# Wendison/FCL-taco2

Measured on AMD Instinct MI355X. Metric: mel-frames/sec (FCL-taco2-S forward, batch=32, 80-mel), higher is better.
Workload: dtype f32 via bf16x3-split MFMA operands, fp32 accumulate (max-abs 8e-6 on mel vs the reference; FCL_PRECISION=0 = exact fp32 MFMA)

## Files before the change

fcl-taco2_amd/_lib.py:

```python
import ctypes as C
import os

_HERE = os.path.dirname(os.path.abspath(__file__))
LIB_PATH = os.environ.get("FCL_LIB") or os.path.join(_HERE, "libfcl_hip.so")

_P = C.c_void_p
_I = C.c_int
_F = C.c_float
_Z = C.c_size_t


class DecoderWeights(C.Structure):
    _fields_ = [("c", _I), ("p", _I), ("u", _I), ("odim", _I)] + [
        (n, _P) for n in ("prenet_w0", "prenet_b0", "prenet_w1", "prenet_b1", "w0_att", "w0_pre", "w0_pos", "w0_hh", "b0",
                          "w1_ih", "w1_hh", "b1", "wf_h", "wf_att")
    ] + [("zoneout_rate", _F), ("prenet_dropout", _F)] + [
        (n + sfx, _P) for n in ("prenet_w0", "prenet_w1", "w0_pre", "w0_hh", "w1_ih", "w1_hh", "wf_h") for sfx in ("_hi", "_lo")] + [
        (n + "_p", _P) for n in ("w0_att", "wf_att", "w0_pre", "w0_hh", "w1_ih", "w1_hh")] + [("out_act", _I), ("wf_h_ff", _P), ("prenet_w0_ff", _P), ("prenet_w1_ff", _P),
                                                                                           ("w0_pre_ff", _P), ("w0_hh_ff", _P), ("w1_ih_ff", _P), ("w1_hh_ff", _P), ("stream", _P),
                                                                                           ("prenet_layers", _I), ("dlayers", _I), ("prenet_w2", _P), ("prenet_b2", _P), ("w2_ih", _P),
                                                                                           ("w2_hh", _P), ("b2", _P), ("reduction_factor", _I)]


class DecoderIO(C.Structure):
# ... 84 lines not shown
        (n, _P) for n in ("window", "twiddle", "frame_utt", "utt_off", "utt_seed", "s", "p", "fr", "y", "c_prev", "c_out", "u_out")]


class Features(C.Structure):
    _fields_ = [("frames", C.c_int64), ("samples", C.c_int64)] + [(n, C.c_int32) for n in ("n_fft", "hop", "n_utt", "n_mels", "nnz", "reserved")] + [
        (n, _P) for n in ("x", "smp_off", "frame_utt", "utt_off", "window", "twiddle", "fb_lo", "fb_off", "fb_w", "mel_stats", "mel", "energy", "mag_out")]


class Pitch(C.Structure):
    _fields_ = [("frames", C.c_int64), ("samples", C.c_int64)] + [(n, C.c_int32) for n in ("n", "hop", "n_utt", "tau_min", "tau_max", "reserved")] + [
        ("fs", _F), ("threshold", _F)] + [(n, _P) for n in ("x", "smp_off", "frame_utt", "utt_off", "f0", "cmnd_out", "tau_out")]


class Resample(C.Structure):
    _fields_ = [("samples_in", C.c_int64), ("samples_out", C.c_int64)] + [(n, C.c_int32) for n in ("l", "m", "k", "n_utt", "max_out", "reserved")] + [
        (n, _P) for n in ("x", "smp_off_in", "smp_off_out", "table", "y")]


class Evaluate(C.Structure):
    _fields_ = [(n, C.c_int64) for n in ("frames_a", "frames_b", "cells", "path_rows")] + [(n, C.c_int32) for n in ("n_pairs", "d", "max_ta", "max_tb")] + [
        (n, _P) for n in ("a", "b", "a_off", "b_off", "cell_off", "path_off", "workspace")] + [("workspace_bytes", _Z)] + [
        (n, _P) for n in ("path", "path_len", "cost", "pitch_a", "pitch_b", "counts", "sums")]


class Align(C.Structure):
    _fields_ = [(n, C.c_int64) for n in ("frames", "rows", "cells")] + [(n, C.c_int32) for n in ("n_utt", "n_states", "max_t", "max_s", "max_skip", "reserved")] + [
        (n, _P) for n in ("ll", "frame_off", "row_off", "cell_off", "row_state", "row_skip", "workspace")] + [("workspace_bytes", _Z)] + [
        (n, _P) for n in ("frame_row", "row_begin", "row_frames", "score", "ok")]


class StftLoss(C.Structure):
    _fields_ = [("frames", C.c_int64), ("samples", C.c_int64)] + [(n, C.c_int32) for n in ("n_fft", "hop", "n_utt", "accumulate")] + [
        (n, _P) for n in ("x", "y", "smp_off", "frame_utt", "utt_off", "window", "twiddle", "frame_sums", "utt_sums", "coef", "fr", "gx")]


class MelLoss(C.Structure):
    _fields_ = [("frames", C.c_int64), ("samples", C.c_int64)] + [(n, C.c_int32) for n in ("n_fft", "hop", "n_utt", "accumulate", "n_mels", "nnz")] + [
        (n, _P) for n in ("x", "y", "smp_off", "frame_utt", "utt_off", "window", "twiddle", "fb_lo", "fb_off", "fb_w", "bt_off", "bt_ch", "bt_w",
                          "frame_sums", "utt_sums", "coef", "fr", "gx")]


class PwdLayer(C.Structure):
    _fields_ = [("samples", C.c_int64)] + [(n, C.c_int32) for n in ("cin", "cout", "ksize", "dilation")] + [("slope", _F), ("reserved", C.c_int32)] + [
        (n, _P) for n in ("x", "w", "bias", "h", "g", "seg_lo", "seg_hi", "y", "dw", "db", "workspace")] + [("workspace_bytes", _Z)]


class BernoulliSite(C.Structure):
    _fields_ = [("out", _P), ("n", C.c_int64), ("p_one", _F), ("seed", C.c_uint32)]


BERNOULLI_MAX_SITES = 16


class LossTerm(C.Structure):
    _fields_ = [(n, _P) for n in ("a", "b", "b2", "valid", "valid2", "da", "da_planes", "sums", "sums2")] + [
        ("m", C.c_int32), ("c", C.c_int32), ("b_log", C.c_int32), ("b_log_offset", _F), ("w_l1", _F), ("w_mse", _F), ("count", C.c_double),
        ("w_l1_2", _F), ("w_mse_2", _F), ("count2", C.c_double)]


LOSS_MAX_TERMS, SUM_ROWS_MAX = 12, 6


class ProfEntry(C.Structure):
    _fields_ = [("name", C.c_char * 56), ("launches", _I), ("ms", C.c_double), ("flops", C.c_double), ("rows", C.c_double), ("fill_bytes", C.c_double)]


TE_MAX_SITES, TE_MAX_LOSSES = 48, 48
TE_TEACHER, TE_KD_TEACHER, TE_STUDENT = 0, 1, 2


class TeConfig(C.Structure):
    _fields_ = ([(n, C.c_int32) for n in ("role", "idim", "odim", "embed_dim", "econv_layers", "econv_chans", "econv_filts", "eunits", "dunits", "prenet_units",
                                          "postnet_layers", "postnet_chans", "postnet_filts", "dp_layers", "dp_chans", "dp_kernel", "vp_layers", "vp_chans",
                                          "vp_kernel", "ve_kernel")]
                + [(n, _F) for n in ("dropout_rate", "zoneout_rate", "dp_dropout", "vp_dropout", "ve_dropout")]
                + [(n, C.c_int32) for n in ("use_masking", "t_embed_dim", "t_econv_chans", "t_eunits", "t_prenet_units", "t_dunits", "t_postnet_chans", "share_proj",
                                            "distill_output", "distill_encoder", "distill_decoder", "distill_prosody", "accum_grad")]
                + [("seed", C.c_uint32), ("site_tag", C.c_uint32 * TE_MAX_SITES), ("dw_planes_min", C.c_int32), ("pred_stream", C.c_int32),
                   ("late_losses", C.c_int32)])


class TeBatch(C.Structure):
    _fields_ = ([(n, C.c_int32) for n in ("B", "T", "L", "N", "F", "lmax")]
                + [(n, _P) for n in ("xs", "ys", "f0", "energy", "ds", "lens", "e_lo", "e_hi", "f_lo", "f_hi", "src_sorted", "row_of_enc", "cell_frame", "frame_cell",
                                     "prev_frame", "cell_row", "dur", "perm_tb", "cell_row_i64", "enc_pad", "enc_valid", "frame_valid", "cell_valid", "pos4",
                                     "live_rows_host")]
                + [("n_enc", C.c_double), ("n_frames", C.c_double)])


class TeKnowledge(C.Structure):
    _fields_ = [("after", _P), ("before", _P), ("enc", _P * 5), ("dec", _P * 8), ("pro", _P * 5), ("dec_cell_major", C.c_int32)]


SIGNATURES = {
    "fcl_te_create": (_I, [C.POINTER(TeConfig), C.POINTER(_P)]),
    "fcl_te_destroy": (None, [_P]),
    "fcl_te_site_name": (C.c_char_p, [_I]),
    "fcl_te_loss_name": (C.c_char_p, [_I]),
    "fcl_te_bind_param": (_I, [_P, C.c_char_p, _P, _P, C.c_int64]),
    "fcl_te_bind_buffer": (_I, [_P, C.c_char_p, _P]),
    "fcl_te_finalize": (_I, [_P, _P]),
    "fcl_te_params_changed": (_I, [_P]),
    "fcl_te_side_stream": (_P, [_P]),
    "fcl_te_place_streams": (_I, [_P, _P, C.POINTER(C.c_int)]),
    "fcl_te_knowledge": (_I, [_P, C.POINTER(TeBatch), C.c_uint32, C.POINTER(TeKnowledge), _P]),
    "fcl_te_forward_backward": (_I, [_P, C.POINTER(TeBatch), C.POINTER(TeKnowledge), C.c_uint32, _P, _P, _P]),
    "fcl_te_backward_stage": (_I, [_P, _I, _P]),
    "fcl_te_join": (_I, [_P, _P]),
    "fcl_te_last_launches": (C.c_int64, [_P]),
    "fcl_te_phase_ms": (_I, [_P, _P]),
    "fcl_te_arena_bytes": (C.c_int64, [_P]),
    "fcl_last_error": (C.c_char_p, []),
    "fcl_version": (_I, []),
    "fcl_debug_ptr": (_P, []),
    "fcl_set_gemm_mode": (_I, [_I]),
    "fcl_get_gemm_mode": (_I, []),
    "fcl_pack_conv1d_weight": (_I, [_P, _P, _P, _I, _I, _I, _P]),
    "fcl_fold_batchnorm": (_I, [_P, _P, _P, _P, _F, _P, _P, _I, _P]),
    "fcl_copy2d": (_I, [_P, _I, _P, _I, _I, _I, _P]),
    "fcl_add2d": (_I, [_P, _I, _P, _I, _I, _I, _F, _P, _P]),
    "fcl_frag_bf16_elems": (_Z, [_I, _I]),
    "fcl_pack_frag_bf16": (_I, [_P, _I, _I, _P, _P, _P]),
    "fcl_pack_frag_f32": (_I, [_P, _I, _I, _P, _P]),
    "fcl_add_vec": (_I, [_P, _P, _P, _I, _P]),
    "fcl_u32_add": (_I, [_P, C.c_uint32, _P]),
    "fcl_planes_elems": (_Z, [_I, _I]),
    "fcl_pack_planes": (_I, [_P, _I, _I, _I, _P, _P]),
    "fcl_linear_planes_fwd": (_I, [_P, _I, _P, _P, _P, _I, _P, _I, _I, _I, _I, _P]),
    "fcl_linear_planes_mse_fwd": (_I, [_P, _I, _P, _P, _I, _P, C.c_double, _P, _I, _P, _P, _I, _I, _I, _P]),
    "fcl_conv1d_planes_fwd": (_I, [_P, _I, _P, _P, _P, _P, _P, _P, _P, _I, _I, _I, _I, _I, _P]),
    "fcl_conv1d_planes_rows_fwd": (_I, [_P, _I, _P, _P, _P, _P, _P, _P, _P, _I, _I, _I, _I, _I, _P, _P]),
    "fcl_embedding_fwd": (_I, [_P, _P, _P, _P, _I, _I, _I, _P]),
    "fcl_embed_conv_table_fwd": (_I, [_P] * 8 + [_I, _I, _I, _I, _I, _P, _P]),
    "fcl_linear_fwd": (_I, [_P, _I, _P, _I, _P, _P, _I, _I, _I, _I, _I, _P]),
    "fcl_conv1d_fwd": (_I, [_P, _P, _P, _P, _P, _P, _P, _I, _I, _I, _I, _I, _P]),
    "fcl_layernorm_fwd": (_I, [_P, _P, _P, _F, _P, _P, _P, _P, _P, _P, _F, _P, _I, _I, _P]),
    "fcl_layernorm_group_fwd": (_I, [_P, _I, C.c_int64, _P, _P, _F, _P, _P, _P, _P, _P, _P, _I, _I, _I, _P]),
    "fcl_conv1d_planes_bn_fwd": (_I, [_P, _I, _P, _P, _P, _P, _I, _I, _I, _I, C.c_float, C.c_float, _P, _P, _P, _P, _P, _P]),
    "fcl_conv1d_planes_group_fwd": (_I, [_P, _I, C.c_int64, _P, _P, _P, _P, _P, _P, _I, _I, _I, _I, _I, _I, _P]),
    "fcl_duration_round_fwd": (_I, [_P, _P, _I, _I, _F, _P, _P]),
    "fcl_variance_embed_add_fwd": (_I, [_P] * 12 + [_I, _I, _I, _P]),
    "fcl_duration_round_ctl_fwd": (_I, [_P, _P, _I, _I, _F, _P, _P, _I, _I, _P]),
    "fcl_variance_embed_add_ctl_fwd": (_I, [_P] * 10 + [_I, _I] + [_P] * 5 + [_I, _I, _I, _P]),
    "fcl_variance_embed_rows_fwd": (_I, [_P] * 11 + [_I, _I] + [_P] * 3 + [_I, _I, _I, _I, _P]),
    "fcl_position_table_fwd": (_I, [_P, _P, _I, _I, _P]),
    "fcl_concat_spk_fwd": (_I, [_P, _I, _P, _P, _P, _I, _I, _I, _I, _P]),
    "fcl_kaldi_ark_append": (C.c_longlong, [_I, C.c_longlong, _I, _P, _P, _P, _I, _P]),
    "fcl_host_device_ptr": (_P, [_P]),
    "fcl_feed_copy": (_I, [_P, _P, _Z, _P, _P, _P, _P]),
    "fcl_row_maps_build": (_I, [C.POINTER(RowMaps), _P]),
    "fcl_gather_rows_fwd": (_I, [_P, _P, _P, _P, _I, _I, _P]),
    "fcl_bilstm_workspace_bytes": (_Z, [_I, _I, _I]),
    "fcl_bilstm_fwd": (_I, [_P] * 13 + [_I, _I, _I, _I, _I, _P, _Z, _P, _P, _P]),
    "fcl_decoder_loop_workspace_bytes": (_Z, [C.POINTER(DecoderWeights), _I]),
    "fcl_decoder_stream_bytes": (_Z, [C.POINTER(DecoderWeights)]),
    "fcl_decoder_stream_pack": (_I, [C.POINTER(DecoderWeights), _P, _Z, _P]),
    "fcl_decoder_loop_fwd": (_I, [C.POINTER(DecoderWeights), C.POINTER(DecoderIO), _P]),
    "fcl_masked_l1_mse_fwd": (_I, [_P, _I, _P, _I, _P, _I, _I, _I, _F, _P, _P]),
    "fcl_gemm_tn_fwd": (_I, [_P, _I, _P, _I, _P, _I, _I, _I, _I, _I, _P, _P, _P]),
    "fcl_gemm_tn_taps_fwd": (_I, [_P, _I, _P, _I, _P, _I, _I, _I, _I, _I, _I, _Z, _P, _P, _P]),
    "fcl_colsum_fwd": (_I, [_P, _P, _P, _P, _P, _I, _I, _I, _P]),
    "fcl_colsum2_fwd": (_I, [_P, _P, _P, _P, _P, _P, _I, _I, _I, _P]),
    "fcl_conv1d_in1_dw": (_I, [_P, _I, _P, _P, _P, _P, _P, _I, _I, _I, _P]),
    "fcl_act_fwd": (_I, [_P, _P, _F, _P, _P, _I, _Z, _I, _P]),
    "fcl_unpack_conv1d_grad": (_I, [_P, _P, _P, _I, _I, _I, _P]),
    "fcl_act_bwd": (_I, [_P, _P, _P, _F, _P, _P, _I, _Z, _I, _P]),
    "fcl_l1_mse_grad": (_I, [_P, _P, _P, _I, _I, _I, _F, _F, _F, C.c_double, _P, _I, _P]),
    "fcl_l1_mse_loss_grad": (_I, [_P, _P, _P, _I, _I, _I, _F, _F, _F, C.c_double, _P, _I, _P, _P, _P]),
    "fcl_layernorm_bwd": (_I, [_P, _P, _P, _F, _P, _P, _P, _P, _P, _F, _P, _P, _P, _P, _P, _I, _I, _P]),
    "fcl_bn_stats_fwd": (_I, [_P, _I, _I, _F, _F, _P, _P, _P, _P, _P, _P]),
    "fcl_bn_stats_ws_fwd": (_I, [_P, _I, _I, _F, _F, _P, _P, _P, _P, _P, _P]),
    "fcl_bn_act_fwd": (_I, [_P, _P, _P, _P, _P, _P, _F, _P, _P, _P, _I, _I, _I, _P]),
    "fcl_bn_bwd": (_I, [_P, _P, _P, _P, _P, _P, _P, _P, _P, _I, _I, _P, _P, _P]),
    "fcl_scale": (_I, [_P, _Z, _F, _P]),
    "fcl_bernoulli_u8": (_I, [_P, _Z, _F, C.c_uint32, _P, _P]),
    "fcl_bernoulli_batch": (_I, [C.POINTER(BernoulliSite), _I, _P]),
    "fcl_lstm_cell_bwd": (_I, [_P, _P, _P, _P, _P, _I, _P, _F, _P, _P, _P, _I, _P, _P, _P, _P, _I, _I, _P]),
    "fcl_scatter_add_rows": (_I, [_P, _P, _P, _I, _I, C.c_int64, _P]),
    "fcl_transpose2d": (_I, [_P, _P, _I, _I, _P]),
    "fcl_pack_planes_t": (_I, [_P, _I, _I, _I, _I, _I, _P, _P, _P, _P]),
    "fcl_gemm_tn_planes": (_I, [_P, _P, _P, _I, _I, _I, _I, _I, _Z, _P]),
    "fcl_pwg_upsample_stage": (_I, [_P, _P, _P, C.c_int64, _I, _I, _P, _P, _P, _I, _I, _P]),
    "fcl_pwg_noise": (_I, [_P, C.c_int64, C.c_uint32, _P]),
    "fcl_pwg_aux_coeff": (_I, [_P, C.c_int64, _I, C.c_int64, _P, _P]),
    "fcl_pwg_first_conv": (_I, [_P, _P, _P, _P, _P, C.c_int64, _I, _I, _P]),
    "fcl_pwg_layer_fwd": (_I, [_P, _P]),
    "fcl_pwg_last_fwd": (_I, [_P, _F, _P, _P, _P, _F, _P, _P, _P, C.c_int64, _I, _P]),
    "fcl_pwg_maps_build": (_I, [_P, _P, _I, C.c_int64, _I, _I, _P, _P, _P, _P, _P, _P, _P, _P, _P, _P]),
    "fcl_pwg_gather_pad": (_I, [_P, C.c_int64, _P, _P, C.c_int64, _I, _P, _P]),
    "fcl_pwg_noise_cap": (_I, [_P, C.c_int64, C.c_uint32, _P, _P, _P]),
    "fcl_pwg_first_conv_cap": (_I, [_P, _P, _P, _P, C.c_int64, _I, _P, _P]),
    "fcl_pwg_layer_cap_fwd": (_I, [_P, _P, _P]),
    "fcl_pwg_last_cap_fwd": (_I, [_P, _F, _P, _P, _P, _F, _P, C.c_int64, _I, _P, _P]),
    "fcl_pcm16_fwd": (_I, [_P, _P, C.c_int64, _P, _P, _P]),
    "fcl_hfg_conv_fwd": (_I, [C.POINTER(HfgConv), _P]),
    "fcl_hfg_tconv_fwd": (_I, [C.POINTER(HfgTconv), _P]),
    "fcl_hfg_unit_fwd": (_I, [C.POINTER(HfgUnit), _P]),
    "fcl_hfg_out_fwd": (_I, [_P, _P, _P, _P, _P, _I, _P, C.c_int64, _I, _I, _I, _P]),
    "fcl_hfg_maps_build": (_I, [_P, _P, _I, C.c_int64, _I, _P, _P, _P, _P]),
    "fcl_hfg_conv_cap_fwd": (_I, [C.POINTER(HfgConv), _P, _P]),
    "fcl_hfg_tconv_cap_fwd": (_I, [C.POINTER(HfgTconv), _P, _P]),
    "fcl_hfg_unit_cap_fwd": (_I, [C.POINTER(HfgUnit), _P, _P]),
    "fcl_hfg_out_cap_fwd": (_I, [_P, _P, _P, _P, _P, _I, _P, C.c_int64, _I, _I, _I, _P, _P]),
    "fcl_gl_mel2lin_fwd": (_I, [_P, _P, _P, _P, C.c_int64, _I, _I, _P]),
    "fcl_gl_phase_init": (_I, [C.POINTER(GriffinLim), _P]),
    "fcl_gl_synth_fwd": (_I, [C.POINTER(GriffinLim), _P]),
    "fcl_gl_ola_fwd": (_I, [C.POINTER(GriffinLim), _P]),
    "fcl_gl_analysis_fwd": (_I, [C.POINTER(GriffinLim), _P]),
    "fcl_fx_logmel_fwd": (_I, [C.POINTER(Features), _P]),
    "fcl_fx_segment_mean_fwd": (_I, [_P, _P, _P, _P, _P, _P, _P, C.c_int64, _I, C.c_int64, _I, _P]),
    "fcl_px_yin_fwd": (_I, [C.POINTER(Pitch), _P]),
    "fcl_px_short_run_fwd": (_I, [_P, _P, _P, _P, C.c_int64, _I, _I, _P]),
    "fcl_rs_resample_fwd": (_I, [C.POINTER(Resample), _P]),
    "fcl_ev_dtw_workspace_bytes": (_Z, [C.c_int64, _I]),
    "fcl_ev_cepstra_fwd": (_I, [_P, _P, _P, _P, C.c_int64, _I, _I, _P]),
    "fcl_ev_dtw_fwd": (_I, [C.POINTER(Evaluate), _P]),
    "fcl_ev_path_pitch_fwd": (_I, [C.POINTER(Evaluate), _P]),
    "fcl_al_workspace_bytes": (_Z, [C.c_int64, _I]),
    "fcl_al_loglik_fwd": (_I, [_P, _P, _P, _P, _P, C.c_int64, _I, _I, _P]),
    "fcl_al_viterbi_fwd": (_I, [C.POINTER(Align), _P]),
    "fcl_al_stats_fwd": (_I, [_P, _P, _P, _P, _P, _P, _P, _P, C.c_int64, C.c_int64, _I, _I, _P]),
    "fcl_stl_sums_fwd": (_I, [C.POINTER(StftLoss), _P]),
    "fcl_stl_grad_bwd": (_I, [C.POINTER(StftLoss), _P]),
    "fcl_msl_sums_fwd": (_I, [C.POINTER(MelLoss), _P]),
    "fcl_msl_grad_bwd": (_I, [C.POINTER(MelLoss), _P]),
    "fcl_pwd_dw_workspace_bytes": (_Z, [C.c_int64, _I, _I, _I]),
    "fcl_pwd_layer_fwd": (_I, [C.POINTER(PwdLayer), _P]),
    "fcl_pwd_layer_dx": (_I, [C.POINTER(PwdLayer), _P]),
    "fcl_pwd_layer_dw": (_I, [C.POINTER(PwdLayer), _P]),
    "fcl_derive_blocks": (_I, [_I, _I, _I]),
    "fcl_derive_batch": (_I, [_P, _I, _I, _P]),
    "fcl_sumsq_accum": (_I, [_P, _Z, _P, _P]),
    "fcl_adam_step": (_I, [_P, _P, _P, _P, _Z, _P, _F, _F, _F, _F, _F, _P, _P, _P]),
    "fcl_adam_step_wd": (_I, [_P, _P, _P, _P, _Z, _P, _F, _F, _F, _F, _F, _F, _P, _P, _P]),
    "fcl_lstm_step_fwd": (_I, [C.POINTER(LstmStep), _P]),
    "fcl_decoder_train_workspace_bytes": (_Z, [_I, _I]),
    "fcl_decoder_train_fwd": (_I, [C.POINTER(DecoderTrain), _P]),
    "fcl_decoder_bptt": (_I, [C.POINTER(DecoderBptt), _P]),
    "fcl_bilstm_train_workspace_bytes": (_Z, [_I, _I]),
    "fcl_bilstm_train_fwd": (_I, [C.POINTER(BilstmTrain), _P]),
    "fcl_bilstm_bptt": (_I, [C.POINTER(BilstmBptt), _P]),
    "fcl_loss_terms_batch": (_I, [C.POINTER(LossTerm), _I, _P]),
    "fcl_sum_rows": (_I, [C.POINTER(C.c_void_p), _I, _P, _P, _P, _I, _I, _P]),
    "fcl_bn_bwd_sums": (_I, [_P, _P, _P, _P, _F, _I, _P, _P, _P, _P, _P, _P, _I, _I, _P]),
    "fcl_act_bwd_sum": (_I, [_P, _P, _P, _P, _F, _P, _P, _I, _Z, _I, _P]),
    "fcl_gather_rows_sum_fwd": (_I, [_P, _P, _P, _P, _P, _P, _I, _I, _P]),
    "fcl_linear2_fwd": (_I, [_P, _I, _P, _I, _I, _P, _I, _P, _I, _I, _P, _P, _I, _P, _I, _I, _I, _I, _P]),
    "fcl_stream_create_cus": (_I, [_I, C.POINTER(C.c_void_p)]),
    "fcl_stream_destroy": (_I, [_P]),
    "fcl_streams_share_pipe": (_I, [_P, _P, C.POINTER(C.c_int), C.POINTER(C.c_double)]),
    "fcl_stream_create_apart": (_I, [C.POINTER(C.c_void_p), _I, C.POINTER(C.c_void_p), C.POINTER(C.c_int)]),
    "fcl_prof_enable": (_I, [_I]),
    "fcl_prof_collect": (_I, [C.POINTER(ProfEntry), _I]),
}

ACT_NONE, ACT_RELU, ACT_TANH, ACT_SIGMOID = 0, 1, 2, 3
DROP_NONE, DROP_MASK, DROP_RNG = 0, 1, 2
STATUS_GROUP_TIMEOUT, STATUS_ZERO_DURATION, STATUS_LMAX_CAP, STATUS_FRAMES_CAP, STATUS_ROWS_CAP = 1, 2, 4, 8, 16
STATUS_VOCODER_CAP, STATUS_PCM_NONFINITE = 32, 64

_lib = None


class FclError(RuntimeError):
    pass


def load():
    global _lib
    if _lib is not None:
        return _lib
    if not os.path.exists(LIB_PATH):
        raise FclError(
            "fcl-taco2_amd: %s not found — build it with `python -c 'import __graft_entry__ as g; g.build()'` "
            "or `make -C fcl-taco2_amd/csrc`.  There is no CPU fallback." % LIB_PATH)
    import torch

    lib = C.CDLL(LIB_PATH)
    for name, (res, args) in SIGNATURES.items():
        fn = getattr(lib, name)
        fn.restype = res
        fn.argtypes = args
    if lib.fcl_version() != ABI_VERSION:
        raise FclError("fcl-taco2_amd: %s has ABI revision %d, this package mirrors %d — rebuild it (`make -C fcl-taco2_amd/csrc`)"
                       % (LIB_PATH, lib.fcl_version(), ABI_VERSION))
    _lib = lib
    return lib


def prof_enable(on):
    check(load().fcl_prof_enable(int(on)))


def prof_collect():
    buf = (ProfEntry * 256)()
    n = load().fcl_prof_collect(buf, 256)
    if n < 0:
        check(n)
    return {buf[i].name.decode(): dict(launches=buf[i].launches, ms=buf[i].ms, flops=buf[i].flops, rows=buf[i].rows, fill_bytes=buf[i].fill_bytes) for i in range(n)}


def check(rc):
    if rc != 0:
        msg = load().fcl_last_error()
        raise FclError("libfcl_hip error %d: %s" % (rc, msg.decode("utf-8", "replace") if msg else "?"))
```

fcl-taco2_amd/batching.py:

```python
import collections
import queue
import sys
import threading

import numpy as np

from .prosody import ProsodyControl


def _grown_caps(engine, maps, n_rows, scale=1.3):
    lmax = max(16, int(maps.lmax * 1.5) + 4)
    bounds = np.full(lmax, 1, dtype=np.int32)
    live = np.minimum(n_rows, (maps.live_rows.astype(np.float64) * scale).astype(np.int64) + 32)
    bounds[: maps.lmax] = live
    bounds[maps.lmax :] = live[-1]
    bounds = np.maximum.accumulate(bounds[::-1])[::-1].astype(np.int32)
    return engine.Caps(lmax, (int(maps.n_frames * scale) + 255) // 256 * 256, bounds, tail_from=maps.lmax + 2)


class _ScaledMaps(object):

    def __init__(self, maps, n_ph_cal, n_ph):
        ratio = float(n_ph) / float(max(n_ph_cal, 1))
        self.lmax = int(maps.lmax)
        self.live_rows = np.ceil(np.asarray(maps.live_rows, dtype=np.float64) * ratio).astype(np.int64)
        self.n_frames = int(np.ceil(maps.n_frames * ratio))


def widened_caps(engine, maps, old, n_rows):
    g = _grown_caps(engine, maps, n_rows, scale=1.6)
    lmax = max(g.lmax, old.lmax)
    return engine.Caps(lmax, max(g.frames, old.frames), np.full(lmax, n_rows, np.int32), tail_from=g.tail_from)


class BucketStore(object):

    def __init__(self, engine, batch_size, make, drain, max_buckets, estimate=True, buckets=None, calibration=None, sizing=None):
        self.engine, self.batch_size, self.make, self.drain, self.estimate = engine, batch_size, make, drain, estimate
        self.sizing = sys.modules[__name__] if sizing is None else sizing
        self.max_buckets = max(1, int(max_buckets))
        self.buckets = collections.OrderedDict() if buckets is None else buckets
        self.calibration = [] if calibration is None else calibration
        self.estimated = self.evicted = 0

    def get(self, t_cap, n_ph):
        b = self.buckets.get(t_cap)
        if b is not None:
            self.buckets.move_to_end(t_cap)
            if b.grow is None:
                return b
            self.drain(b)
            del self.buckets[t_cap]
            return self._add(t_cap, self.sizing.widened_caps(self.engine, b.grow, b.caps, self.batch_size * t_cap))
        if not (self.calibration and self.estimate):
            return None
        maps, n_ph_cal = self.calibration[0]
        self.estimated += 1
        return self._add(t_cap, self.sizing._grown_caps(self.engine, self.sizing._ScaledMaps(maps, n_ph_cal, n_ph), self.batch_size * t_cap))

    def calibrated(self, t_cap, maps, n_ph):
        if not self.calibration:
            self.calibration.append((maps, n_ph))
        return self._add(t_cap, self.sizing._grown_caps(self.engine, maps, self.batch_size * t_cap))

    def _add(self, t_cap, caps):
        b = self.buckets[t_cap] = self.make(t_cap, caps)
        while len(self.buckets) > self.max_buckets:
            old_cap, old = next(iter(self.buckets.items()))
            self.drain(old)
            del self.buckets[old_cap]
            self.evicted += 1
        return b


def make_batches(lengths, batch_frames):
    order = sorted(range(len(lengths)), key=lambda i: -lengths[i])
    out, cur, tot = [], [], 0
    for i in order:
        if cur and tot + lengths[i] > batch_frames:
            out.append(cur)
            cur, tot = [], 0
        cur.append(i)
        tot += lengths[i]
    if cur:
        out.append(cur)
    return out


class Writer(object):

    def __init__(self, write, maxsize):
        self._write, self._q, self._err = write, queue.Queue(maxsize=maxsize), []
        self._th = threading.Thread(target=self._run, daemon=True)
        self._th.start()

    def _run(self):
        while True:
            got = self._q.get()
            if got is None:
                return
            item, event = got
            try:
                if not self._err:
                    self._write(item)
            except Exception as e:
                self._err.append(e)
            finally:
                if event is not None:
                    event.set()

    def put(self, item, event=None):
        self._q.put((item, event))

    def join(self):
        if self._th.is_alive():
            self._q.put(None)
            self._th.join()

    def close(self):
        self.join()
        if self._err:
            raise self._err[0]


class NullArk(object):

    def __enter__(self):
        return self

    def __exit__(self, *exc):
        return False

    def write_batch(self, keys, mats, counts):
        pass


def chunk_selectors(plan, utts, prosody):
    has_spk = plan.hp.spk_embed_dim is not None
    if has_spk and any(len(u) < 3 for u in utts):
        raise ValueError("fcl-taco2_amd: the model has spk_embed_dim=%d: every utterance needs a speaker embedding" % plan.hp.spk_embed_dim)
    spk_of = (lambda chunk: [u[2] for u in chunk]) if has_spk else (lambda chunk: None)
    controlled = prosody is not None
    if isinstance(prosody, dict):
        per_utt = {k: ProsodyControl.coerce(v) for k, v in prosody.items()}
        ctl_of = lambda chunk: [per_utt.get(u[0]) for u in chunk]
    elif controlled:
        one = ProsodyControl.coerce(prosody)
        ctl_of = lambda chunk: [one] * len(chunk)
    else:
        ctl_of = lambda chunk: None
    return spk_of, ctl_of, controlled


def take(pending, pred=None):
    for it in [p for p in pending if pred is None or pred(p)]:
        pending.remove(it)
        yield it
```

fcl-taco2_amd/csrc/bilstm.hip:

```cpp
#include <map>
#include <mutex>

#include "fcl_common.h"
#include "row_maps.h"
#include "lstm_epilogue.h"

namespace fcl {



template <int H, bool SAVE = false, bool MAPS = false>
__global__ __launch_bounds__(4 * H) void bilstm_persistent_kernel(const float* __restrict__ gx_f, const float* __restrict__ gx_r,
                                                                   const float* __restrict__ whh_f, const float* __restrict__ whh_r,
                                                                   const int* __restrict__ lens, float* __restrict__ out, int T, BilstmSave sv = BilstmSave(),
                                                                   unsigned short* __restrict__ out_p = nullptr ,
                                                                   fcl_row_maps_t mp = fcl_row_maps_t()) {
    if constexpr (MAPS) {
        if (blockIdx.x == gridDim.x - 1) {
            if (blockIdx.y == 0) {
                row_maps_block<4 * H>(mp);
                row_maps_finish_block<4 * H>(mp);
            }
            return;
        }
    }
    __shared__ __attribute__((aligned(16))) float h_s[H];
    __shared__ float g_s[4 * H];
    const int b = blockIdx.x, dir = blockIdx.y, j = threadIdx.x;
    const float* gx = (dir ? gx_r : gx_f) + (size_t)b * T * (4 * H);
    const float* whh = dir ? whh_r : whh_f;
    const int len = lens[b];

    float w[H];
#pragma unroll
    for (int k = 0; k < H; k += 4) {
        const f32x4 v = *reinterpret_cast<const f32x4*>(whh + (size_t)j * H + k);
        w[k] = v[0]; w[k + 1] = v[1]; w[k + 2] = v[2]; w[k + 3] = v[3];
    }
    if (j < H) h_s[j] = 0.f;
    float c = 0.f;
    for (int t = len + (j / H); t < T; t += 4) {
        out[((size_t)b * T + t) * (2 * H) + dir * H + (j % H)] = 0.f;
        if (out_p) store_p32(out_p, (2 * H + 31) >> 5, b * T + t, dir * H + (j % H), 0.f);
    }
    __syncthreads();

    int t = dir ? len - 1 : 0;
    const int dt = dir ? -1 : 1;
    float gnext = len > 0 ? gx[(size_t)t * (4 * H) + j] : 0.f;
    for (int s = 0; s < len; ++s, t += dt) {
        const float gcur = gnext;
        if (s + 1 < len) gnext = gx[(size_t)(t + dt) * (4 * H) + j];
        float a0 = 0.f, a1 = 0.f, a2 = 0.f, a3 = 0.f;
#pragma unroll
        for (int k = 0; k < H; k += 4) {
            const f32x4 hv = *reinterpret_cast<const f32x4*>(&h_s[k]);
            a0 = fmaf(w[k], hv[0], a0);
            a1 = fmaf(w[k + 1], hv[1], a1);
            a2 = fmaf(w[k + 2], hv[2], a2);
            a3 = fmaf(w[k + 3], hv[3], a3);
        }
        g_s[j] = gcur + ((a0 + a1) + (a2 + a3));
        __syncthreads();
        if (j < H) {
            const float ig = sigmoid_f(g_s[j]), fg = sigmoid_f(g_s[H + j]), gg = tanh_f(g_s[2 * H + j]), og = sigmoid_f(g_s[3 * H + j]);
            if (SAVE) {
                const size_t cell = (size_t)t * sv.B + b;
                float* sg = sv.gates[dir] + cell * (4 * H);
                sg[j] = ig; sg[H + j] = fg; sg[2 * H + j] = gg; sg[3 * H + j] = og;
                sv.c_old[dir][cell * H + j] = c;
                sv.h_old[dir][cell * H + j] = h_s[j];
            }
            c = fg * c + ig * gg;
            if (SAVE) sv.c_new[dir][((size_t)t * sv.B + b) * H + j] = c;
            const float h = og * tanh_f(c);
            h_s[j] = h;
            out[((size_t)b * T + t) * (2 * H) + dir * H + j] = h;
            if (out_p) store_p32(out_p, (2 * H + 31) >> 5, b * T + t, dir * H + j, h);
        }
        __syncthreads();
    }
}

typedef float f32x2 __attribute__((ext_vector_type(2)));
__device__ __forceinline__ void ks_exclusive() {
#ifdef FCL_KS_EXCLUSIVE
    asm volatile("v_mov_b32 v255, 0" ::: "v255");
#endif
}
template <int CTRL>
__device__ __forceinline__ float dpp_f(float v) {
#ifdef FCL_KS_BPERMUTE
    const int lane = (int)__builtin_amdgcn_mbcnt_hi(~0u, __builtin_amdgcn_mbcnt_lo(~0u, 0u));
    const int src = CTRL == 0x141 ? ((lane & ~7) | (7 - (lane & 7))) : CTRL == 0x4E ? (lane ^ 2) : CTRL == 0xB1 ? (lane ^ 1) : CTRL == 0x128 ? ((lane & ~15) | ((lane + 8) & 15))
                    : ((lane & ~3) | (CTRL & 3));
    return __builtin_bit_cast(float, __builtin_amdgcn_ds_bpermute(src << 2, __builtin_bit_cast(int, v)));
#else
    asm volatile("s_nop 3" : "+v"(v));
    return __builtin_bit_cast(float, __builtin_amdgcn_update_dpp(0, __builtin_bit_cast(int, v), CTRL, 0xf, 0xf, true));
#endif
}

__device__ __forceinline__ void ks_matvec(const f32x2 (&w)[4][16], const float* __restrict__ v16, float (&a8)[8]) {
    f32x4 hv[4];
#pragma unroll
    for (int e = 0; e < 4; ++e) hv[e] = *reinterpret_cast<const f32x4*>(v16 + 4 * e);
    f32x2 acc[4] = {f32x2{0.f, 0.f}, f32x2{0.f, 0.f}, f32x2{0.f, 0.f}, f32x2{0.f, 0.f}};
#pragma unroll
    for (int kk = 0; kk < 16; ++kk) {
        const float hk = hv[kk >> 2][kk & 3];
#pragma unroll
        for (int p = 0; p < 4; ++p) acc[p] = __builtin_elementwise_fma(w[p][kk], f32x2{hk, hk}, acc[p]);
    }
#pragma unroll
    for (int p = 0; p < 4; ++p) {
        a8[2 * p] = acc[p][0];
        a8[2 * p + 1] = acc[p][1];
    }
}

__device__ __forceinline__ float ks_reduce_scatter8(const float (&a8)[8], int q3) {
    const bool lo1 = q3 < 4, lo2 = (q3 & 2) == 0, lo3 = (q3 & 1) == 0;
    float k4[4];
#pragma unroll
    for (int x = 0; x < 4; ++x) k4[x] = (lo1 ? a8[x] : a8[4 + x]) + dpp_f<0x141>(lo1 ? a8[4 + x] : a8[x]);
    float k2[2];
#pragma unroll
    for (int x = 0; x < 2; ++x) k2[x] = (lo2 ? k4[x] : k4[2 + x]) + dpp_f<0x4E>(lo2 ? k4[2 + x] : k4[x]);
    return (lo3 ? k2[0] : k2[1]) + dpp_f<0xB1>(lo3 ? k2[1] : k2[0]);
}

struct KsCell {
    float a, c_new, h;
};
__device__ __forceinline__ KsCell ks_cell(float z, int g, float c) {
    const float sc = g == 2 ? 2.f : 1.f;
    const float r = __builtin_amdgcn_rcpf(1.0f + __expf(-sc * z));
    KsCell o;
    o.a = g == 2 ? 2.0f * r - 1.0f : r;
    const float ig = dpp_f<0x00>(o.a), fg = dpp_f<0x55>(o.a), gg = dpp_f<0xAA>(o.a), og = dpp_f<0xFF>(o.a);
    o.c_new = fg * c + ig * gg;
    o.h = og * tanh_f(o.c_new);
    return o;
}

template <bool SAVE = false, bool MAPS = false>
__global__ __launch_bounds__(512) void bilstm_ksplit_kernel(const float* __restrict__ gx_f, const float* __restrict__ gx_r,
                                                            const float* __restrict__ whh_f, const float* __restrict__ whh_r,
                                                            const int* __restrict__ lens, float* __restrict__ out, int T, BilstmSave sv = BilstmSave(),
                                                            unsigned short* __restrict__ out_p = nullptr, fcl_row_maps_t mp = fcl_row_maps_t()) {
    constexpr int H = 128;
    if constexpr (MAPS) {
        if (blockIdx.x == gridDim.x - 1) {
            if (blockIdx.y == 0) {
                row_maps_block<4 * H>(mp);
                row_maps_finish_block<4 * H>(mp);
            }
            return;
        }
    }
    __shared__ __attribute__((aligned(16))) float h_s[2][H];
    ks_exclusive();
    const int b = blockIdx.x, dir = blockIdx.y, j = threadIdx.x;
    const int q = j & 7, R = j >> 3;
    const int g = q & 3, U = 2 * R + (q >> 2);
    const float* gx = (dir ? gx_r : gx_f) + (size_t)b * T * (4 * H);
    const float* whh = dir ? whh_r : whh_f;
    const int len = lens[b];

    f32x2 w[4][16];
#pragma unroll
    for (int p = 0; p < 4; ++p) {
        const float* r0 = whh + (size_t)(((2 * p) & 3) * H + 2 * R + ((2 * p) >> 2)) * H + 16 * q;
        const float* r1 = whh + (size_t)(((2 * p + 1) & 3) * H + 2 * R + ((2 * p + 1) >> 2)) * H + 16 * q;
#pragma unroll
        for (int kk = 0; kk < 16; kk += 4) {
            const f32x4 v0 = *reinterpret_cast<const f32x4*>(r0 + kk), v1 = *reinterpret_cast<const f32x4*>(r1 + kk);
#pragma unroll
            for (int e = 0; e < 4; ++e) w[p][kk + e] = f32x2{v0[e], v1[e]};
        }
    }
    if (j < 2 * H) (&h_s[0][0])[j] = 0.f;
    for (int t = len + (j / H); t < T; t += 4) {
        out[((size_t)b * T + t) * (2 * H) + dir * H + (j % H)] = 0.f;
        if (out_p) store_p32(out_p, (2 * H + 31) >> 5, b * T + t, dir * H + (j % H), 0.f);
    }
    __syncthreads();

    const int t0 = dir ? len - 1 : 0, dt = dir ? -1 : 1;
    const float* gp = gx + g * H + U;
    float gq[4];
#pragma unroll
    for (int d = 0; d < 4; ++d) gq[d] = d < len ? gp[(size_t)(t0 + d * dt) * (4 * H)] : 0.f;
    float c = 0.f, h_prev = 0.f;

    for (int s0 = 0; s0 < len; s0 += 4) {
#pragma unroll
        for (int d = 0; d < 4; ++d) {
            const int s = s0 + d;
            if (s >= len) break;
            const int t = t0 + s * dt;
            const float gcur = gq[d];
            if (s + 4 < len) gq[d] = gp[(size_t)(t + 4 * dt) * (4 * H)];
            float a8[8];
            ks_matvec(w, h_s[d & 1] + 16 * q, a8);
            const KsCell cl = ks_cell(gcur + ks_reduce_scatter8(a8, q), g, c);
            const float a = cl.a, c_new = cl.c_new, h = cl.h;
            if (SAVE) {
                const size_t cell = (size_t)t * sv.B + b;
                sv.gates[dir][cell * (4 * H) + g * H + U] = a;
                if (g == 0) {
                    sv.c_old[dir][cell * H + U] = c;
                    sv.h_old[dir][cell * H + U] = h_prev;
                    sv.c_new[dir][cell * H + U] = c_new;
                }
            }
            if (g == 0) {
                h_s[(d & 1) ^ 1][U] = h;
                out[((size_t)b * T + t) * (2 * H) + dir * H + U] = h;
                if (out_p) store_p32(out_p, (2 * H + 31) >> 5, b * T + t, dir * H + U, h);
            }
            c = c_new;
            h_prev = h;
            __syncthreads();
        }
    }
}

template <int H>
__global__ __launch_bounds__(4 * H) void bilstm_bptt_persistent_kernel(BilstmBwd a, const int* __restrict__ lens, int T) {
    __shared__ __attribute__((aligned(16))) float dg_s[4 * H];
    __shared__ float p_s[4][H];
    const int b = blockIdx.x, dir = blockIdx.y, j = threadIdx.x;
    const int q = j / H, k = j % H;
    const int len = lens[b];
    float w[H];
    const float* wt = a.whh_t[dir] + (size_t)k * (4 * H) + q * H;
#pragma unroll
    for (int r = 0; r < H; r += 4) {
        const f32x4 v = *reinterpret_cast<const f32x4*>(wt + r);
        w[r] = v[0]; w[r + 1] = v[1]; w[r + 2] = v[2]; w[r + 3] = v[3];
    }
    float* dg = a.dg[dir];
    for (int t = len; t < T; ++t) dg[((size_t)t * a.B + b) * (4 * H) + j] = 0.f;
    float dh = 0.f, dc = 0.f;
    int t = dir ? 0 : len - 1;
    const int dt = dir ? 1 : -1;
    for (int s = 0; s < len; ++s, t += dt) {
        const size_t cell = (size_t)t * a.B + b;
        if (j < H) {
            const float* g = a.gates[dir] + cell * (4 * H);
            const float ig = g[j], fg = g[H + j], gg = g[2 * H + j], og = g[3 * H + j];
            const float dho = dh + a.d_out[((size_t)b * T + t) * a.ld + dir * H + j];
            const float tc = tanh_f(a.c_new[dir][cell * H + j]);
            const float dcn = dc + dho * og * (1.0f - tc * tc);
            const float d0 = dcn * gg * ig * (1.0f - ig), d1 = dcn * a.c_old[dir][cell * H + j] * fg * (1.0f - fg);
            const float d2 = dcn * ig * (1.0f - gg * gg), d3 = dho * tc * og * (1.0f - og);
            dg_s[j] = d0; dg_s[H + j] = d1; dg_s[2 * H + j] = d2; dg_s[3 * H + j] = d3;
            float* o = dg + cell * (4 * H);
            o[j] = d0; o[H + j] = d1; o[2 * H + j] = d2; o[3 * H + j] = d3;
            dc = dcn * fg;
        }
        __syncthreads();
        float a0 = 0.f, a1 = 0.f, a2 = 0.f, a3 = 0.f;
#pragma unroll
        for (int r = 0; r < H; r += 4) {
            const f32x4 dv = *reinterpret_cast<const f32x4*>(&dg_s[q * H + r]);
            a0 = fmaf(w[r], dv[0], a0);
            a1 = fmaf(w[r + 1], dv[1], a1);
            a2 = fmaf(w[r + 2], dv[2], a2);
            a3 = fmaf(w[r + 3], dv[3], a3);
        }
        p_s[q][k] = (a0 + a1) + (a2 + a3);
        __syncthreads();
        if (j < H) dh = (p_s[0][j] + p_s[1][j]) + (p_s[2][j] + p_s[3][j]);
    }
}

__global__ __launch_bounds__(512) void bilstm_bptt_ksplit_kernel(BilstmBwd a, const int* __restrict__ lens, int T) {
    constexpr int H = 128;
    __shared__ __attribute__((aligned(16))) float dg_s[2][4 * H];
    ks_exclusive();
    const int b = blockIdx.x, dir = blockIdx.y, j = threadIdx.x;
    const int rs = j & 31, q3 = rs & 7, kg = j >> 5;
    const bool owner = rs < 8;
    const int u = 8 * kg + q3;
    const int len = lens[b];
    f32x2 w[4][16];
#pragma unroll
    for (int pr = 0; pr < 4; ++pr) {
        const float* c0 = a.whh_t[dir] + (size_t)(8 * kg + 2 * pr) * (4 * H) + 16 * rs;
        const float* c1 = c0 + 4 * H;
#pragma unroll
        for (int rr = 0; rr < 16; rr += 4) {
            const f32x4 v0 = *reinterpret_cast<const f32x4*>(c0 + rr), v1 = *reinterpret_cast<const f32x4*>(c1 + rr);
#pragma unroll
            for (int e = 0; e < 4; ++e) w[pr][rr + e] = f32x2{v0[e], v1[e]};
        }
    }
    float* dg = a.dg[dir];
    for (int t = len; t < T; ++t) dg[((size_t)t * a.B + b) * (4 * H) + j] = 0.f;
    float dh = 0.f, dc = 0.f;
    const int t0 = dir ? 0 : len - 1, dt = dir ? 1 : -1;
    float pre[7] = {0.f, 0.f, 0.f, 0.f, 0.f, 0.f, 0.f};
    auto fetch = [&](int t) {
        const size_t cell = (size_t)t * a.B + b;
        const float* gsv = a.gates[dir] + cell * (4 * H);
        pre[0] = gsv[u]; pre[1] = gsv[H + u]; pre[2] = gsv[2 * H + u]; pre[3] = gsv[3 * H + u];
        pre[4] = a.d_out[((size_t)b * T + t) * a.ld + dir * H + u];
        pre[5] = a.c_new[dir][cell * H + u];
        pre[6] = a.c_old[dir][cell * H + u];
    };
    if (owner && len > 0) fetch(t0);
    for (int s0 = 0; s0 < len; s0 += 2) {
#pragma unroll
        for (int d = 0; d < 2; ++d) {
            const int s = s0 + d;
            if (s >= len) break;
            const int t = t0 + s * dt;
            if (owner) {
                const float ig = pre[0], fg = pre[1], gg = pre[2], og = pre[3], dout = pre[4], cn = pre[5], co = pre[6];
                if (s + 1 < len) fetch(t + dt);
                const float dho = dh + dout;
                const float tc = tanh_f(cn);
                const float dcn = dc + dho * og * (1.0f - tc * tc);
                const float d0 = dcn * gg * ig * (1.0f - ig), d1 = dcn * co * fg * (1.0f - fg);
                const float d2 = dcn * ig * (1.0f - gg * gg), d3 = dho * tc * og * (1.0f - og);
                float* ds = dg_s[d];
                ds[u] = d0; ds[H + u] = d1; ds[2 * H + u] = d2; ds[3 * H + u] = d3;
                float* o = dg + ((size_t)t * a.B + b) * (4 * H);
                o[u] = d0; o[H + u] = d1; o[2 * H + u] = d2; o[3 * H + u] = d3;
                dc = dcn * fg;
            }
            __syncthreads();
            if (s + 1 < len) {
                float a8[8];
                ks_matvec(w, dg_s[d] + 16 * rs, a8);
                float v = ks_reduce_scatter8(a8, q3);
                v += dpp_f<0x128>(v);
                v += __builtin_bit_cast(float, __builtin_amdgcn_ds_swizzle(__builtin_bit_cast(int, v), 0x401F));
                dh = v;
            }
        }
    }
}

struct GroupSync {
    unsigned int* flag;
    unsigned int* error;
};

__device__ __forceinline__ void xchg_store(float* p, float v) { __hip_atomic_store(p, v, __ATOMIC_RELAXED, __HIP_MEMORY_SCOPE_AGENT); }
__device__ __forceinline__ float xchg_load(const float* p) { return __hip_atomic_load(p, __ATOMIC_RELAXED, __HIP_MEMORY_SCOPE_AGENT); }

__device__ __forceinline__ bool group_barrier(const GroupSync& gs, int group, unsigned int target) {
    __builtin_amdgcn_s_waitcnt(0);
    __syncthreads();
    __shared__ int ok_s;
    if (threadIdx.x == 0) {
        __hip_atomic_fetch_add(gs.flag + group, 1u, __ATOMIC_RELAXED, __HIP_MEMORY_SCOPE_AGENT);
        int ok = 0;
        for (long long spin = 0; spin < (1ll << 24); ++spin) {
            if (__hip_atomic_load(gs.flag + group, __ATOMIC_RELAXED, __HIP_MEMORY_SCOPE_AGENT) >= target) { ok = 1; break; }
        }
        if (!ok) atomicOr(gs.error, (unsigned int)FCL_STATUS_GROUP_TIMEOUT);
        ok_s = ok;
    }
    __syncthreads();
    return ok_s != 0;
}

template <bool SAVE>
__global__ __launch_bounds__(512) void bilstm_group_kernel(const float* __restrict__ gx_f, const float* __restrict__ gx_r, const float* __restrict__ whh_f,
// ... 443 lines not shown
        FCL_BILSTM_CASE(128)
    }
#undef FCL_BILSTM_CASE
    return false;
}

}

extern "C" {

size_t fcl_bilstm_workspace_bytes(int b, int t, int h) {
    if (b <= 0 || t <= 0 || h <= 0) return 0;
    return sizeof(float) * ((size_t)2 * b * t * 4 * h + (size_t)6 * b * h) + 256 + (h == 256 ? bilstm_group_workspace_bytes(b, h) : 0);
}

int fcl_bilstm_fwd(const float* x, const int32_t* lens, const float* w_ih_f, const float* w_hh_f, const float* b_f,
                   const float* w_ih_r, const float* w_hh_r, const float* b_r, float* out, uint16_t* out_p, const uint16_t* x_p,
                   const uint16_t* w_ih_f_p, const uint16_t* w_ih_r_p, int b, int t, int c, int h,
                   int algo, void* workspace, size_t workspace_bytes, uint32_t* status, const fcl_row_maps_t* row_maps, fcl_stream_t stream) {
    FCL_REQUIRE((x || x_p) && lens && w_ih_f && w_hh_f && b_f && w_ih_r && w_hh_r && b_r && out, FCL_ERR_INVALID, "bilstm_fwd: null argument");
    FCL_REQUIRE((x_p == nullptr) == (w_ih_f_p == nullptr) && (x_p == nullptr) == (w_ih_r_p == nullptr), FCL_ERR_INVALID,
                "bilstm_fwd: x_p / w_ih_f_p / w_ih_r_p come together");
    FCL_REQUIRE(x || x_p, FCL_ERR_INVALID, "bilstm_fwd: no input");
    FCL_REQUIRE(b > 0 && t > 0 && c > 0 && h > 0 && (c & 3) == 0 && (h & 3) == 0, FCL_ERR_SHAPE, "bilstm_fwd: bad sizes B=%d T=%d C=%d H=%d", b, t, c, h);
    FCL_REQUIRE(workspace && workspace_bytes >= fcl_bilstm_workspace_bytes(b, t, h), FCL_ERR_WORKSPACE, "bilstm_fwd: workspace too small");
    FCL_REQUIRE(aligned16(workspace) && aligned16(out), FCL_ERR_ALIGN, "bilstm_fwd: 16-byte alignment required");
    bool maps_fusable = false;
    if (row_maps) {
        const int rc = row_maps_check(row_maps, &maps_fusable);
        if (rc) return rc;
    }
    hipStream_t s = (hipStream_t)stream;
    float* gx_f = reinterpret_cast<float*>(workspace);
    float* gx_r = gx_f + (size_t)b * t * 4 * h;
    float* hbuf = gx_r + (size_t)b * t * 4 * h;
    float* cbuf = hbuf + (size_t)4 * b * h;

    for (int d = 0; d < 2; ++d) {
        GemmArgs g = {};
        g.term[0] = GemmTerm{x, d ? w_ih_r : w_ih_f, c, c, c, 0};
        if (x_p && w_ih_f_p && w_ih_r_p) {
            g.term[0].Ap = x_p;
            g.term[0].Wp = d ? w_ih_r_p : w_ih_f_p;
            g.term[0].lda_p = g.term[0].ldw_p = (c + 31) / 32;
        }
        g.nterms = 1;
        g.M = b * t;
        g.N = 4 * h;
        g.bias = d ? b_r : b_f;
        g.Y = d ? gx_r : gx_f;
        g.ldy = 4 * h;
        int rc = launch_gemm(g, s);
        if (rc) return rc;
    }
    const bool can_persist = (h == 8 || h == 16 || h == 32 || h == 64 || h == 128);
    static const int group_infer = tunable("BILSTM_GROUP_INFER", 0);
    FCL_REQUIRE(algo != 3 || status, FCL_ERR_INVALID, "bilstm_fwd: algo 3 (cooperating workgroups) needs a device status word");
    struct MapsAfter {
        const fcl_row_maps_t* m;
        fcl_stream_t st;
        int finish(int rc) const { return (rc || !m) ? rc : fcl_row_maps_build(m, st); }
    } after{row_maps, stream};
    if (h == 256 && status && (algo == 3 || (algo == 0 && group_infer))) {
        void* gws = hbuf;
        const size_t gbytes = workspace_bytes - sizeof(float) * ((size_t)2 * b * t * 4 * h);
        if (launch_bilstm_group(gx_f, gx_r, w_hh_f, w_hh_r, lens, out, b, t, h, nullptr, gws, gbytes, status, s)) {
            FCL_HIP(hipGetLastError());
            return after.finish(out_p ? fcl_pack_planes(out, 2 * h, b * t, 2 * h, out_p, stream) : 0);
        }
    }
    if (algo == 0 || algo == 3) algo = can_persist ? 2 : 1;
    FCL_REQUIRE(algo == 1 || (algo == 2 && can_persist), FCL_ERR_INVALID, "bilstm_fwd: algo %d unavailable for H=%d", algo, h);
    const bool fuse_wanted = row_maps && maps_fusable;
    if (algo == 2 && h == 128 &&
        (fuse_wanted ? ks_claims_simd(bilstm_ksplit_kernel<false, true>, "bilstm_ksplit_kernel<false, true>")
                     : ks_claims_simd(bilstm_ksplit_kernel<false, false>, "bilstm_ksplit_kernel<false, false>"))) {
        const bool fuse = fuse_wanted;
        ProfScope ps(fuse ? "bilstm_ksplit_kernel+maps" : "bilstm_ksplit_kernel", 2.0 * 2 * b * (double)t * 4 * h * h, (double)b * t, s);
        if (fuse)
            hipLaunchKernelGGL((bilstm_ksplit_kernel<false, true>), dim3(b + 1, 2), dim3(512), 0, s, gx_f, gx_r, w_hh_f, w_hh_r, lens, out, t, BilstmSave(), out_p,
                               *row_maps);
        else
            hipLaunchKernelGGL((bilstm_ksplit_kernel<false, false>), dim3(b, 2), dim3(512), 0, s, gx_f, gx_r, w_hh_f, w_hh_r, lens, out, t, BilstmSave(), out_p,
                               fcl_row_maps_t());
        const int rc = check_hip(hipGetLastError(), "bilstm k-split launch");
        return fuse ? rc : after.finish(rc);
    }
    if (algo == 2 && h == 128 && fuse_wanted) {
        ProfScope ps("bilstm_persistent_kernel+maps", 2.0 * 2 * b * (double)t * 4 * h * h, (double)b * t, s);
        hipLaunchKernelGGL((bilstm_persistent_kernel<128, false, true>), dim3(b + 1, 2), dim3(512), 0, s, gx_f, gx_r, w_hh_f, w_hh_r, lens, out, t, BilstmSave(),
                           out_p, *row_maps);
        return check_hip(hipGetLastError(), "bilstm persistent (+ row maps) launch");
    }
    if (algo == 2) {
        ProfScope ps("bilstm_persistent_kernel", 2.0 * 2 * b * (double)t * 4 * h * h, (double)b * t, s);
        dim3 grid(b, 2);
#define FCL_BILSTM_CASE(HH) \
    case HH: hipLaunchKernelGGL((bilstm_persistent_kernel<HH>), grid, dim3(4 * HH), 0, s, gx_f, gx_r, w_hh_f, w_hh_r, lens, out, t, BilstmSave(), out_p); break;
        switch (h) {
            FCL_BILSTM_CASE(8)
            FCL_BILSTM_CASE(16)
            FCL_BILSTM_CASE(32)
            FCL_BILSTM_CASE(64)
            FCL_BILSTM_CASE(128)
        }
#undef FCL_BILSTM_CASE
        return after.finish(check_hip(hipGetLastError(), "bilstm persistent launch"));
    }
    hipLaunchKernelGGL(fill_kernel, dim3(64), dim3(256), 0, s, hbuf, (long long)6 * b * h, 0.f);
    auto step_args = [&](int d, int st, int cur) {
        float* hp[2] = {hbuf + (size_t)d * b * h, hbuf + (size_t)(2 + d) * b * h};
        const int tt = d ? t - 1 - st : st;
        LstmStepArgs a = {};
        a.term[0] = GemmTerm{hp[cur], d ? w_hh_r : w_hh_f, h, h, h, 0};
        a.nterms = 1;
        a.M = b;
        a.U = h;
        a.G = d ? gx_r : gx_f;
        a.g_row_mul = t;
        a.g_row_add = tt;
        a.step = tt;
        a.h_in = hp[cur];
        a.h_out = hp[cur ^ 1];
        a.c = cbuf + (size_t)d * b * h;
        a.zoneout = 0.f;
        a.row_len = lens;
        a.out2 = out;
        a.out2_row_mul = t;
        a.out2_row_add = tt;
        a.ld2 = 2 * h;
        a.out2_col_off = d * h;
        return a;
    };
    if (lstm_step_is_small(b, h)) {
        int cur = 0;
        for (int st = 0; st < t; ++st) {
            int rc = launch_lstm_small_pair(step_args(0, st, cur), step_args(1, st, cur), s);
            if (rc) return rc;
            cur ^= 1;
        }
    } else {
        for (int d = 0; d < 2; ++d) {
            int cur = 0;
            for (int st = 0; st < t; ++st) {
                int rc = launch_lstm_step(step_args(d, st, cur), s);
                if (rc) return rc;
                cur ^= 1;
            }
        }
    }
    return after.finish(out_p ? fcl_pack_planes(out, 2 * h, b * t, 2 * h, out_p, stream) : 0);
}

}
```

fcl-taco2_amd/decode.py:

```python
import argparse
import collections
import importlib
import json
import logging
import os
import sys
import threading
import time

import numpy as np
import torch

from .batching import BucketStore, NullArk, Writer, _grown_caps, _ScaledMaps, chunk_selectors, take, widened_caps
from .kaldi_io import ArkScpWriter
from .prosody import FIELDS as PROSODY_FIELDS, ProsodyControl
from .sharding import shard_utterances

MODULE_MAP = {
    "nets.teacher_training.e2e_tts_tacotron2_sa": "fcl_taco2_amd.nets.teacher_training.e2e_tts_tacotron2_sa",
    "nets.knowledge_distillation.e2e_tts_tacotron2_sa_kd_student": "fcl_taco2_amd.nets.knowledge_distillation.e2e_tts_tacotron2_sa_kd_student",
    "nets.knowledge_distillation.e2e_tts_tacotron2_sa_kd_teacher": "fcl_taco2_amd.nets.knowledge_distillation.e2e_tts_tacotron2_sa_kd_teacher",
}


# ... 38 lines not shown
    for k, v in js.items():
        ids = np.array(list(map(int, v["output"][0]["tokenid"].split())), dtype=np.int64)
        if len(v.get("input", [])) > 1 and "feat" in v["input"][1] and v["input"][1].get("filetype") != "npy":
            from .kaldi_io import read_vec

            path, off = v["input"][1]["feat"].rsplit(":", 1)
            utts.append((k, ids, read_vec(path, int(off))))
        else:
            utts.append((k, ids))
    return utts


class _Slot(object):

    def __init__(self, frames_cap, odim, batch, slab=None):
        if slab is None:
            slab = torch.empty(self.words(frames_cap, odim, batch), dtype=torch.float32, pin_memory=True)
        self.whole = slab[: self.words(frames_cap, odim, batch)]
        n = frames_cap * odim
        self.mel = slab[:n].view(frames_cap, odim)
        self.f0 = slab[n : n + batch + 1].view(torch.int32)
        self.st = slab[n + batch + 1 : n + batch + 2].view(torch.int32)
        self.free = threading.Event()
        self.free.set()

    @staticmethod
    def words(frames_cap, odim, batch):
        from .engine import packed_words

        return packed_words(frames_cap, odim, batch)


class _Pool(object):

    def __init__(self, plan, batch, t_cap, caps, streams, seed, controls=False):
        self.plan, self.batch, self.caps, self.t_cap, self.streams, self.seed = plan, batch, caps, t_cap, streams, seed
        self.controls = controls
        self.runners, self.slots, self.next, self.grow = [None] * len(streams), [None] * len(streams), 0, None
        self._slab = None

    def runner(self, j):
        from . import engine

        if self.runners[j] is None:
            pools_ = self.plan.__dict__.setdefault("_decode_cache", {}).setdefault("graph_mempools", {})
            mp = pools_.setdefault(self.streams[j].cuda_stream, torch.cuda.graph_pool_handle()) if SHARE_GRAPH_POOLS else None
            r = self.runners[j] = engine.BatchRunner(self.plan, self.batch, self.t_cap, self.caps, forced=False, stream=self.streams[j], seed=self.seed + 7919 * j,
                                                     pack_outputs=True, mempool=mp, controls=self.controls)
            odim = int(r.mel.shape[1])
            w = _Slot.words(self.caps.frames, odim, self.batch)
            if self._slab is None:
                self._slab = torch.empty(2 * len(self.streams) * w, dtype=torch.float32, pin_memory=True)
            self.slots[j] = [_Slot(self.caps.frames, odim, self.batch, self._slab[(2 * j + q) * w : (2 * j + q + 1) * w]) for q in range(2)]
        return self.runners[j]

    def retire(self):
        shared = self.plan.__dict__.get("_decode_cache", {}).get("graph_mempools", {})
        for j, r in enumerate(self.runners):
            if r is not None:
                shared.pop(self.streams[j].cuda_stream, None)


grown_caps, ScaledMaps = _grown_caps, _ScaledMaps


SHARE_GRAPH_POOLS = os.environ.get("FCL_DECODE_SHARE_POOLS", "1") not in ("", "0")
ESTIMATE_CAPS = os.environ.get("FCL_DECODE_ESTIMATE_CAPS", "1") not in ("", "0")
MAX_BUCKETS = 8


def release_graphs(model_or_plan):
    plan = model_or_plan.plan() if hasattr(model_or_plan, "plan") and callable(model_or_plan.plan) else model_or_plan
    plan.__dict__.pop("_decode_cache", None)


@torch.no_grad()
def decode(model, utts, out_prefix, batch_size=32, seed=137, depth=4, stats=None, keep_graphs=True, max_buckets=None, prosody=None):
    from . import engine, ops

    torch.manual_seed(seed)
    order = sorted(range(len(utts)), key=lambda i: -len(utts[i][1]))
    dev = next(model.parameters()).device
    plan = model.plan(dev)
    spk_of, ctl_of, controlled = chunk_selectors(plan, utts, prosody)
    ckey = ("ctl",) if controlled else ()
    frames = 0
    depth = max(1, int(depth))
    cache = plan.__dict__.setdefault("_decode_cache", {})
    streams = engine.shared_streams(dev, depth)
    pending = []
    n_eager = n_graph = n_redo = 0
    eager_only = bool(getattr(plan, "generic_decoder", False)) or plan.hp.elayers != 1

    def eager(chunk):
        prep = engine.prepare(plan, [u[1] for u in chunk], spembs=spk_of(chunk), prosody=ctl_of(chunk))
        mel, utt_frames, inter = engine.run(plan, prep, ops.DROP_RNG, seed=int(torch.randint(0, 2 ** 31 - 1, (1,)).item()), return_intermediates=True)
        arr = mel.cpu().numpy()
        wr.put((chunk, arr, list(utt_frames)))
        return int(arr.shape[0]), inter["maps"]

    def harvest(item):
        nonlocal n_redo
        pool, j, chunk, slot, ev = item
        ev.synchronize()
        if int(slot.st[0]) != 0:
            pool.runners[j].status.zero_()
            slot.free.set()
            n_redo += 1
            got, pool.grow = eager(chunk)
            return got
        f0 = slot.f0.numpy()
        total = int(f0[len(chunk)])
        wr.put((chunk, slot.mel.numpy()[:total], [int(v) for v in np.diff(f0[: len(chunk) + 1])]), slot.free)
        return total

    def drain(pool):
        nonlocal frames
        for it in take(pending, lambda p: p[0] is pool):
            frames += harvest(it)
        for sl in [x for pair in pool.slots if pair for x in pair]:
            sl.free.wait()
        pool.retire()

    store = BucketStore(engine, batch_size, lambda t_cap, caps: _Pool(plan, batch_size, t_cap, caps, streams, seed + 31 * bi, controlled), drain,
                        MAX_BUCKETS if max_buckets is None else max_buckets, ESTIMATE_CAPS,
                        cache.setdefault(("pools", batch_size, depth) + ckey, collections.OrderedDict()), cache.setdefault(("calibration", batch_size) + ckey, []),
                        sizing=sys.modules[__name__])
    with (ArkScpWriter(out_prefix) if out_prefix is not None else NullArk()) as w, torch.cuda.device(dev):
        wr = Writer(lambda it: w.write_batch([u[0] for u in it[0]], it[1][: int(sum(it[2]))], it[2]), 4 * (depth + 1))
        torch.cuda.synchronize()
        t0 = time.perf_counter()
        try:
            for bi, s in enumerate(range(0, len(order), batch_size)):
                chunk = [utts[i] for i in order[s : s + batch_size]]
                if eager_only:
                    got, _ = eager(chunk)
                    frames += got
                    n_eager += 1
                    continue
                t_cap = (max(len(u[1]) for u in chunk) + 15) // 16 * 16
                n_ph = sum(len(u[1]) for u in chunk)
                pool = store.get(t_cap, n_ph)
                if pool is None:
                    got, maps = eager(chunk)
                    frames += got
                    n_eager += 1
                    store.calibrated(t_cap, maps, n_ph)
                    continue
                j = pool.next % len(streams)
                pool.next += 1
                for it in take(pending, lambda p: p[1] == j):
                    frames += harvest(it)
                r = pool.runner(j)
                slot = pool.slots[j][(pool.next // len(streams)) % 2]
                slot.free.wait()
                slot.free.clear()
                try:
                    r.load([u[1] for u in chunk], spembs=spk_of(chunk), prosody=ctl_of(chunk))
                except Exception:
                    slot.free.set()
                    raise
                r.replay()
                with torch.cuda.stream(r.stream):
                    if r.out is not None and r.out.numel() == slot.whole.numel():
                        slot.whole.copy_(r.out, non_blocking=True)
                    else:
                        slot.mel.copy_(r.mel, non_blocking=True)
                        slot.f0.copy_(r._frames.utt_frame0, non_blocking=True)
                        slot.st.copy_(r.status, non_blocking=True)
                    ev = torch.cuda.Event()
                    ev.record(r.stream)
                pending.append((pool, j, chunk, slot, ev))
                n_graph += 1
            while pending:
                frames += harvest(pending.pop(0))
            torch.cuda.synchronize()
            dev_secs = time.perf_counter() - t0
        except BaseException:
            torch.cuda.synchronize()
            for it in take(pending):
                it[0].runners[it[1]].status.zero_()
                it[3].free.set()
            raise
        finally:
            wr.join()
            if not keep_graphs:
                release_graphs(plan)
        secs = time.perf_counter() - t0
        wr.close()
    if stats is not None:
        stats.update(device_seconds=dev_secs, eager_batches=n_eager, graph_batches=n_graph, redone_batches=n_redo, buckets=len(store.buckets),
                     evicted_buckets=store.evicted, estimated_buckets=store.estimated)
    return frames, secs


def add_prosody_arguments(ap):
    g = ap.add_argument_group("prosody control (edits the predicted durations / pitch / energy; INTEGRATION.md)")
    g.add_argument("--duration-scale", type=float, default=None, help="speaking-rate factor on the predicted durations, in (0, 8] (2: twice as long)")
    g.add_argument("--pitch-scale", type=float, default=None, help="scale of the normalised pitch")
    g.add_argument("--pitch-shift", type=float, default=None, help="shift of the normalised pitch")
    g.add_argument("--energy-scale", type=float, default=None, help="scale of the normalised energy")
    g.add_argument("--energy-shift", type=float, default=None, help="shift of the normalised energy")
    g.add_argument("--semitones", type=float, default=None, help="pitch shift in semitones (needs --f0-en-stats)")
    g.add_argument("--pitch-range", type=float, default=None, help="pitch-range factor (same as --pitch-scale)")
    g.add_argument("--energy-gain", type=float, default=None, help="energy gain on the linear energy (needs --f0-en-stats)")
    g.add_argument("--f0-en-stats", default=None, help="f0_en_stats.npy of preprocessing: [f0_mean, f0_std, en_mean, en_std]")
    g.add_argument("--prosody-json", default=None, help="per-utterance controls {utt_id: {field: value}} on top of the global ones")


def prosody_from_args(args, utt_ids=None):
    raw = {f: getattr(args, f) for f in PROSODY_FIELDS if getattr(args, f) is not None}
    units = {k: getattr(args, k) for k in ("semitones", "pitch_range", "energy_gain") if getattr(args, k) is not None}
    if ("semitones" in units or "pitch_range" in units) and ("pitch_scale" in raw or "pitch_shift" in raw):
        raise ValueError("--semitones / --pitch-range and --pitch-scale / --pitch-shift both set the pitch control: give one of them")
    if "energy_gain" in units and ("energy_scale" in raw or "energy_shift" in raw):
        raise ValueError("--energy-gain and --energy-scale / --energy-shift both set the energy control: give one of them")
    if ("semitones" in units or "energy_gain" in units) and args.f0_en_stats is None:
        raise ValueError("--semitones / --energy-gain need --f0-en-stats (the pitch / energy statistics of preprocessing)")
    base = dict(raw)
    if units:
        u = ProsodyControl.from_units(stats=args.f0_en_stats, semitones=units.get("semitones", 0.0), pitch_range=units.get("pitch_range", 1.0),
                                      energy_gain=units.get("energy_gain", 1.0))
        if "semitones" in units or "pitch_range" in units:
            base.update(pitch_scale=u.pitch_scale, pitch_shift=u.pitch_shift)
        if "energy_gain" in units:
            base.update(energy_scale=u.energy_scale, energy_shift=u.energy_shift)
    glob = ProsodyControl(**base)
    if args.prosody_json is None:
        return glob if base else None
    with open(args.prosody_json) as f:
        per = json.load(f)
    if not isinstance(per, dict) or not all(isinstance(v, dict) for v in per.values()):
        raise ValueError("--prosody-json: expected {utt_id: {field: value}}")
    out = {k: ProsodyControl.coerce(dict(base, **v)) for k, v in per.items()}
    for k in (utt_ids or ()):
        out.setdefault(k, glob)
    return out


def main(argv=None):
    ap = argparse.ArgumentParser(description="FCL-taco2 mel synthesis on MI355X (reference-compatible decode driver)")
    ap.add_argument("--model", required=True)
    ap.add_argument("--model-conf", required=True)
    ap.add_argument("--teacher-config", default=None, help="model.json of the teacher (student checkpoints trained with KD projections)")
    ap.add_argument("--json", required=True)
    ap.add_argument("--out", required=True)
    ap.add_argument("--batch-size", type=int, default=32)
    ap.add_argument("--nj", type=int, default=1, help="number of utterance shards (one process per GPU)")
    ap.add_argument("--job", type=int, default=0, help="this process's shard (0-based)")
    ap.add_argument("--seed", type=int, default=137)
    ap.add_argument("--verbose", type=int, default=1)
    add_prosody_arguments(ap)
    args = ap.parse_args(argv)
    try:
        prosody_from_args(args)
    except ValueError as e:
        ap.error(str(e))
    torch.set_num_threads(4)
    logging.basicConfig(level=logging.INFO if args.verbose else logging.WARN, format="%(asctime)s %(levelname)s: %(message)s")
    dev = "cuda:%d" % (args.job % max(torch.cuda.device_count(), 1))
    model = build_model(args.model, args.model_conf, args.teacher_config, dev)
    utts = read_manifest(args.json)
    mine = shard_utterances([len(u[1]) for u in utts], args.nj)[args.job]
    out = args.out if args.nj == 1 else "%s.%d" % (args.out, args.job + 1)
    prosody = prosody_from_args(args, [utts[i][0] for i in mine])
    frames, secs = decode(model, [utts[i] for i in mine], out, args.batch_size, args.seed, prosody=prosody)
    logging.info("average inference speed = %.1f frames / sec. (%d utterances, %d frames)", frames / max(secs, 1e-9), len(mine), frames)
    return frames, secs


if __name__ == "__main__":
    main()
```

fcl-taco2_amd/engine.py:

```python
import os
import time

import numpy as np
import torch

from . import ops
from . import prosody as _prosody
from .hparams import output_act_code
from .plan import LN_EPS


class RowMaps(object):
    __slots__ = ("src_rows", "order", "dur_sorted", "frame_off_sorted", "live_rows", "utt_frames", "n_frames", "lmax",
                 "frame_lo", "frame_hi")


def build_row_maps(lens, durs, t_max, frames_per_step=1):
    B = len(lens)
    lens_np = np.asarray(lens, dtype=np.int64)
    parts = [np.asarray(d).reshape(-1) for d in durs]
    for b in range(B):
        assert parts[b].shape[0] == lens_np[b], "duration count != phoneme count"
    dur = np.concatenate(parts).astype(np.int64) if B else np.zeros(0, dtype=np.int64)
    assert (dur > 0).all(), "zero duration: ds_nonzeros.shape[0] != hs.shape[0]"
    n = dur.shape[0]
    starts = np.zeros(B + 1, dtype=np.int64)
    np.cumsum(lens_np, out=starts[1:])
    src = np.arange(n, dtype=np.int64) + np.repeat(np.arange(B, dtype=np.int64) * t_max - starts[:-1], lens_np)
    csum = np.cumsum(dur) * int(frames_per_step)
    foff = csum - dur * int(frames_per_step)
    fstarts = np.zeros(B + 1, dtype=np.int64)
    fstarts[1:] = csum[starts[1:] - 1]
    utt = fstarts[1:] - fstarts[:-1]
    order = np.argsort(-dur, kind="stable")
    m = RowMaps()
    m.order = order
    m.src_rows = src[order].astype(np.int32)
    m.dur_sorted = dur[order].astype(np.int32)
    m.frame_off_sorted = foff[order].astype(np.int32)
    m.lmax = int(m.dur_sorted[0])
    m.live_rows = np.ascontiguousarray((n - np.cumsum(np.bincount(dur, minlength=m.lmax + 1))[: m.lmax]).astype(np.int32))
    m.utt_frames = [int(v) for v in utt]
    m.n_frames = int(fstarts[-1])
    m.frame_lo = np.repeat(fstarts[:-1], utt).astype(np.int32)
    m.frame_hi = np.repeat(fstarts[1:], utt).astype(np.int32)
    return m


def _predictor_scalar(pp, hs, seg_lo, seg_hi, pad_mask_u8):
    x = hs
    n = len(pp.convs)
    out = None
    for i, cv in enumerate(pp.convs):
        x = ops.conv1d(x, cv.wp, cv.bias, seg_lo, seg_hi, ops.ACT_RELU)
        last = i == n - 1
        x, out = ops.layernorm(x, pp.ln[i][0], pp.ln[i][1], LN_EPS, want_y=not last,
                               lin_w=pp.lin_w if last else None, lin_b=pp.lin_b if last else None,
                               pad_mask=pad_mask_u8 if last else None)
    return out


def _predictor_scalar_planes(pp, hs_p, seg_lo, seg_hi, pad_mask_u8):
    xp = hs_p
    n = len(pp.convs)
    out = None
    for i, cv in enumerate(pp.convs):
        y, _ = ops.conv1d_planes(xp, cv, seg_lo, seg_hi, ops.ACT_RELU, want_f32=True, want_planes=False)
        last = i == n - 1
        if last:
            _, out = ops.layernorm(y, pp.ln[i][0], pp.ln[i][1], LN_EPS, want_y=False, lin_w=pp.lin_w, lin_b=pp.lin_b, pad_mask=pad_mask_u8)
        else:
            _, _, xp = ops.layernorm(y, pp.ln[i][0], pp.ln[i][1], LN_EPS, want_y=False, want_planes=True)
    return out


def _predictors_grouped(grp, hs_p, seg_lo, seg_hi, pad_u8, m, masked):
    G, C = grp.G, grp.chans
    y, _ = ops.conv1d_planes(hs_p, grp.w0, seg_lo, seg_hi, ops.ACT_RELU, want_f32=True, want_planes=False)
    ldx, gstride = G * C, C
    out = None
    for i in range(grp.layers):
        last = i == grp.layers - 1
        if last:
            same_mask = all(masked) or not any(masked)
            assert same_mask, "grouped predictors share one pad-mask policy"
            _, out, _ = ops.layernorm_group(y, ldx, gstride, grp.gamma[i], grp.beta[i], LN_EPS, m, C, G, lin_w=grp.lin_w, lin_b=grp.lin_b,
                                            pad_mask=pad_u8 if all(masked) else None)
        else:
            _, _, xp = ops.layernorm_group(y, ldx, gstride, grp.gamma[i], grp.beta[i], LN_EPS, m, C, G, want_planes=True)
            y, _ = ops.conv1d_planes_group(xp, m * (C // 32) * 64, grp.wpp[i], grp.bias[i], seg_lo, seg_hi, m, C, C, grp.k, G, act=ops.ACT_RELU)
            ldx, gstride = C, m * C
    return [out[g * m : (g + 1) * m] for g in range(G)]


def use_planes(plan):
    hp = plan.hp
    if getattr(plan, "generic_decoder", False) or hp.elayers != 1:
        return False
    return (ops.planes_enabled() and plan.enc_convs[0].wpp is not None and plan.decoder.struct.w0_att_p is not None
            and all(x % 32 == 0 for x in (hp.embed_dim, hp.econv_chans, hp.eunits, hp.adim, hp.postnet_chans, hp.duration_predictor_chans,
                                          hp.variance_predictor_chans)))


class PreparedBatch(object):
    __slots__ = ("B", "T", "lens", "ids", "seg_lo", "seg_hi", "pad", "lens_dev", "f0e", "maps", "src_rows", "dur", "frame_off",
                 "frame_lo", "frame_hi", "dur_pad", "spk", "ctl")


class Caps(object):
    __slots__ = ("lmax", "frames", "bounds", "tail_from")

    def __init__(self, lmax, frames, bounds, tail_from=0):
        self.lmax, self.frames = int(lmax), int(frames)
        self.bounds = np.ascontiguousarray(np.asarray(bounds, dtype=np.int32))
        self.tail_from = int(tail_from) if 0 < int(tail_from) < self.lmax else 0
        assert self.bounds.shape == (self.lmax,) and self.lmax > 0 and self.frames > 0

    @staticmethod
    def from_maps(maps):
        return Caps(maps.lmax, maps.n_frames, maps.live_rows)

    @staticmethod
    def for_batches(host_maps, slack_steps=0, frame_round=256):
        lmax = max(m.lmax for m in host_maps) + int(slack_steps)
        bounds = np.ones(lmax, dtype=np.int32)
        for m in host_maps:
            bounds[: m.lmax] = np.maximum(bounds[: m.lmax], m.live_rows)
        return Caps(lmax, (max(m.n_frames for m in host_maps) + frame_round - 1) // frame_round * frame_round, bounds)

    @staticmethod
    def generous(n_rows, lmax, frames):
        return Caps(lmax, frames, np.full(lmax, n_rows, dtype=np.int32))


class DeviceFrames(object):

    def __init__(self, maps, caps, device, status=None):
        self.utt_frame0, self.totals, self.live_rows, self.caps, self.device = maps["utt_frame0"], maps["totals"], maps["live_rows"], caps, device
        self.status = status
        self._host = None

    def resolve(self):
        if self._host is None:
            if self.status is None:
                ops.check_status(self.device)
            else:
                bits = int(self.status.item()) & 0xFFFFFFFF
                if bits:
                    self.status.zero_()
                    raise ops._lib.FclError("fcl-taco2_amd: device status 0x%x: %s" % (bits, ops.status_message(bits)))
            f0 = self.utt_frame0.cpu().numpy()
            self._host = [int(v) for v in (f0[1:] - f0[:-1])]
        return self._host


_RING = None
import os as _os

_GROUP_PREDICTORS = _os.environ.get("FCL_PRED_GROUP", "1") not in ("", "0")
_VAR_EMBED_ROWS = _os.environ.get("FCL_VAR_EMBED_ROWS", "1") not in ("", "0")


def _ring():
    global _RING
    if _RING is None:
        from .hostio import PinnedRing

        _RING = PinnedRing(depth=8)
    return _RING


def _upload_maps(holder, maps, dev):
    holder.maps = maps
    blocks = dict(src_rows=maps.src_rows, dur=maps.dur_sorted, frame_off=maps.frame_off_sorted, frame_lo=maps.frame_lo, frame_hi=maps.frame_hi)
    layout, off = {}, 0
    for k, v in blocks.items():
        layout[k] = (off, v.size)
        off += (v.size + 3) // 4 * 4
    i32 = np.zeros(off, dtype=np.int32)
    for k, v in blocks.items():
        i32[layout[k][0] : layout[k][0] + v.size] = v
    with torch.cuda.device(dev):
        up = _ring().upload({"i32m": torch.from_numpy(i32)}, dev)["i32m"]
    for k, (o, n) in layout.items():
        setattr(holder, k, up[o : o + n])


def prepare(plan, xs, durs=None, f0=None, energy=None, device_maps=False, spembs=None, prosody=None):
    dev = plan.device
    p = PreparedBatch()
    p.B = len(xs)
    p.lens = [int(len(x)) for x in xs]
    p.T = T = max(p.lens)
    controls = _prosody.per_utterance(prosody, p.B)
    _prosody.check_overrides(controls, forced_dur=durs is not None, forced_f0e=f0 is not None)
    ids = np.zeros((p.B, T), dtype=np.int64)
    for b, x in enumerate(xs):
        ids[b, : p.lens[b]] = x.cpu().numpy() if torch.is_tensor(x) else np.asarray(x)
    lens_np = np.asarray(p.lens, dtype=np.int64)
    rows = np.arange(p.B * T, dtype=np.int64)
    b_of = rows // T
    blocks = {"seg_lo": (b_of * T).astype(np.int32), "seg_hi": (b_of * T + lens_np[b_of]).astype(np.int32), "lens_dev": lens_np.astype(np.int32)}
    p.maps, p.dur_pad = None, None
    if durs is not None and device_maps:
        dpad = np.zeros((p.B, T), dtype=np.int32)
        for b in range(p.B):
            d = np.asarray(durs[b]).reshape(-1)
            assert d.shape[0] == p.lens[b], "duration count != phoneme count"
            dpad[b, : p.lens[b]] = d
        blocks["dur_pad"] = dpad.reshape(-1)
    elif durs is not None:
        p.maps = m = build_row_maps(p.lens, durs, T, plan.hp.reduction_factor)
        blocks.update(src_rows=m.src_rows, dur=m.dur_sorted, frame_off=m.frame_off_sorted, frame_lo=m.frame_lo, frame_hi=m.frame_hi)
    layout, off = {}, 0
    for k, v in blocks.items():
        layout[k] = (off, v.size)
        off += (v.size + 3) // 4 * 4
    i32 = np.zeros(off, dtype=np.int32)
    for k, v in blocks.items():
        i32[layout[k][0] : layout[k][0] + v.size] = v
    items = {"ids": torch.from_numpy(ids.reshape(-1)), "i32": torch.from_numpy(i32),
             "pad": torch.from_numpy(((rows % T) >= lens_np[b_of]).astype(np.uint8))}
    if f0 is not None:
        pe = np.zeros((2, p.B, T), dtype=np.float32)
        for b in range(p.B):
            pe[0, b, : p.lens[b]] = np.asarray(f0[b]).reshape(-1)
            pe[1, b, : p.lens[b]] = np.asarray(energy[b]).reshape(-1)
        items["f0e"] = torch.from_numpy(pe.reshape(2, -1))
    if controls is not None:
        items["ctl"] = torch.from_numpy(_prosody.pack(controls, p.lens, T))
    if plan.hp.spk_embed_dim is not None:
        if spembs is None:
            raise ValueError("fcl-taco2_amd: the model was built with spk_embed_dim=%d: every utterance needs its speaker embedding" % plan.hp.spk_embed_dim)
        sp = np.stack([(s.detach().cpu().numpy() if torch.is_tensor(s) else np.asarray(s)).reshape(-1) for s in spembs]).astype(np.float32)
        assert sp.shape == (p.B, plan.hp.spk_embed_dim), "speaker embeddings must be [B, spk_embed_dim]"
        items["spk"] = torch.from_numpy(np.ascontiguousarray(sp))
    elif spembs is not None:
        raise ValueError("fcl-taco2_amd: speaker embeddings given to a model without spk_embed_dim")
    with torch.cuda.device(dev):
        up = _ring().upload(items, dev)
    p.ids, p.pad, p.f0e, p.spk, p.ctl = up["ids"], up["pad"], up.get("f0e"), up.get("spk"), up.get("ctl")
    for k, (o, n) in layout.items():
        setattr(p, k, up["i32"][o : o + n])
    return p


def encode(plan, prep, bilstm_algo=0, planes=False, row_maps=None):
    bl = plan.blstm
    res = plan.hp.use_residual
    convs, tabs = plan.enc_convs, getattr(plan, "embed_conv_tables", None)
    if tabs is not None:
        x, xp = ops.embed_conv_table(prep.ids, tabs, convs[0].bias, prep.seg_lo, prep.seg_hi, ops.ACT_RELU, residual_table=plan.embed if res else None,
                                     want_f32=res or not planes, want_planes=planes)
        convs = convs[1:]
    if planes:
        if tabs is None:
            x, xp = ops.embedding(prep.ids, plan.embed, want_f32=res, want_planes=True)
        for cv in convs:
            x, xp = ops.conv1d_planes(xp, cv, prep.seg_lo, prep.seg_hi, ops.ACT_RELU, residual=x if res else None, want_f32=res)
        return ops.bilstm(None, prep.lens_dev, bl["w_ih_f"], bl["w_hh_f"], bl["b_f"], bl["w_ih_r"], bl["w_hh_r"], bl["b_r"], prep.B, prep.T, bilstm_algo,
                          x_p=xp, w_ih_p=(bl["w_ih_p_f"], bl["w_ih_p_r"]), want_planes=True, row_maps=row_maps)
    if tabs is None:
        x = ops.embedding(prep.ids, plan.embed)
    for cv in convs:
        x = ops.conv1d(x, cv.wp, cv.bias, prep.seg_lo, prep.seg_hi, ops.ACT_RELU, residual=x if res else None)
    for i, bl in enumerate(plan.blstm_layers):
        x = ops.bilstm(x, prep.lens_dev, bl["w_ih_f"], bl["w_hh_f"], bl["b_f"], bl["w_ih_r"], bl["w_hh_r"], bl["b_r"], prep.B, prep.T, bilstm_algo,
                       row_maps=row_maps if i == 0 else None)
    return x


class _DevMaps(object):

    def __init__(self, dm, caps):
        self.src_rows, self.dur, self.frame_off, self.frame_lo, self.frame_hi = dm["src_rows"], dm["dur"], dm["frame_off"], dm["frame_lo"], dm["frame_hi"]
        self.live_dev, self.live_rows, self.n_frames, self.lmax = dm["live_rows"], caps.bounds, caps.frames, caps.lmax
        self.tail_from = caps.tail_from
        self.order = None


def run(plan, prep, dropout_mode=ops.DROP_RNG, prenet_keep=None, seed=0, bilstm_algo=0, return_intermediates=False, seed_dev=None, caps=None,
        status=None):
    hp, dev = plan.hp, plan.device
    with torch.cuda.device(dev):
        planes = use_planes(plan)
        hs_p = None
        maps_req = None
        if prep.maps is None and prep.dur_pad is not None and caps is not None:
            maps_req = ops.row_maps_request(prep.B * prep.T, prep.B, caps.lmax, caps.frames, dur_i32=prep.dur_pad, t_max=prep.T, pad=prep.pad,
                                            status=status)
        if planes:
            hs, hs_p = encode(plan, prep, bilstm_algo, planes=True, row_maps=maps_req)
            predictor = lambda pp, pad: _predictor_scalar_planes(pp, hs_p, prep.seg_lo, prep.seg_hi, pad)
        else:
            hs = encode(plan, prep, bilstm_algo, row_maps=maps_req)
            predictor = lambda pp, pad: _predictor_scalar(pp, hs, prep.seg_lo, prep.seg_hi, pad)
        inter = {"hs": hs, "T": prep.T} if return_intermediates else None
        if hp.spk_embed_dim is not None:
            if getattr(prep, "spk", None) is None:
                raise ValueError("fcl-taco2_amd: this pass needs speaker embeddings (prepare(..., spembs=...))")
            hs, hs_p = ops.concat_spk(hs, prep.spk, prep.T, want_f32=True, want_planes=planes)
        rm = prep
        frames_info = None
        ctl = getattr(prep, "ctl", None)
        grouped = planes and prep.f0e is None and _GROUP_PREDICTORS
        m_rows = prep.B * prep.T
        p = e = None
        if prep.maps is None:
            d_int = None
            if prep.dur_pad is None:
                if grouped and plan.group_dpe is not None:
                    d_log, p, e = _predictors_grouped(plan.group_dpe, hs_p, prep.seg_lo, prep.seg_hi, prep.pad, m_rows, [True, True, True])
                else:
                    d_log = predictor(plan.duration, None)
                if ctl is not None:
                    d_int = ops.duration_round_ctl(d_log, ctl, 1, False, 1.0, prep.pad)
                else:
                    d_int = ops.duration_round(d_log, False, 1.0, prep.pad)
                if inter is not None:
                    inter["d_log"], inter["d_int"] = d_log, d_int
            if caps is not None:
                dm = maps_req.maps if maps_req is not None else ops.row_maps_build(prep.B * prep.T, prep.B, caps.lmax, caps.frames, dur_i64=d_int,
                                                                                   t_max=prep.T, pad=prep.pad, status=status)
                rm = PreparedBatch()
                rm.maps = _DevMaps(dm, caps)
                rm.src_rows, rm.dur, rm.frame_off, rm.frame_lo, rm.frame_hi = dm["src_rows"], dm["dur"], dm["frame_off"], dm["frame_lo"], dm["frame_hi"]
                frames_info = DeviceFrames(dm, caps, dev, status)
            else:
                if d_int is None:
                    raise ValueError("prepare(device_maps=True) leaves the row maps to the device: run() needs caps")
                d_host = d_int.cpu().numpy().reshape(prep.B, prep.T)
                rm = PreparedBatch()
                _upload_maps(rm, build_row_maps(prep.lens, [d_host[b, : prep.lens[b]] for b in range(prep.B)], prep.T, hp.reduction_factor), dev)
        if prep.f0e is not None:
            p, e = prep.f0e[0], prep.f0e[1]
        elif p is None and grouped and plan.group_pe is not None:
            p, e = _predictors_grouped(plan.group_pe, hs_p, prep.seg_lo, prep.seg_hi, prep.pad, m_rows, [True, True])
        elif p is None:
            p = predictor(plan.pitch, prep.pad)
            e = predictor(plan.energy, prep.pad)
        att_c = att_c_p = None
        if planes and _VAR_EMBED_ROWS and not return_intermediates and hs.shape[1] % 32 == 0 and plan.pitch_embed_wt.shape[0] <= 31:
            p_emb = e_emb = None
            att_c_p, p_c, e_c = ops.variance_embed_rows(hs, p, e, plan.pitch_embed_wt, plan.pitch_embed_b, plan.energy_embed_wt, plan.energy_embed_b,
                                                        prep.seg_lo, prep.seg_hi, rm.src_rows, ctl, 1, want_scalars=ctl is not None)
            if ctl is not None:
                p, e = p_c, e_c
        elif ctl is not None:
            att, p_emb, e_emb, p, e = ops.variance_embed_add_ctl(hs, p, e, plan.pitch_embed_w, plan.pitch_embed_b, plan.energy_embed_w,
                                                                 plan.energy_embed_b, prep.seg_lo, prep.seg_hi, ctl, 1, want_embs=return_intermediates)
        else:
            att, p_emb, e_emb = ops.variance_embed_add(hs, p, e, plan.pitch_embed_w, plan.pitch_embed_b, plan.energy_embed_w,
                                                       plan.energy_embed_b, prep.seg_lo, prep.seg_hi, want_embs=return_intermediates)
        maps = rm.maps
        if att_c_p is None:
            att_c, att_c_p = (ops.gather_rows(att, rm.src_rows, want_f32=False, want_planes=True) if planes else (ops.gather_rows(att, rm.src_rows), None))
        keep_dev = None
        if hp.dropout_rate <= 0.0:
            dropout_mode = ops.DROP_NONE
        if dropout_mode == ops.DROP_MASK and maps.order is None:
            raise ValueError("injected prenet masks are given in (utterance, phoneme) order: they need host-built row maps")
        if dropout_mode == ops.DROP_MASK:
            keep = np.ascontiguousarray(np.asarray(prenet_keep)[: maps.lmax][:, :, maps.order, :])
            keep_dev = torch.from_numpy(keep).to(dev)
        before = ops.decoder_loop(plan.decoder, att_c, rm.dur, maps.live_rows, rm.frame_off, maps.n_frames,
                                  dropout_mode=dropout_mode, prenet_keep=keep_dev, seed=seed, seed_dev=seed_dev, att_c_p=att_c_p, want_before_p=planes,
                                  live_rows_dev=getattr(maps, "live_dev", None), status=status, tail_from=getattr(maps, "tail_from", 0))
        n_post = len(plan.postnet)
        if planes:
            before, xp = before
            f_dev = frames_info.totals[:1] if frames_info is not None else None
            for i, cv in enumerate(plan.postnet):
                last = i == n_post - 1
                x, xp = ops.conv1d_planes(xp, cv, rm.frame_lo, rm.frame_hi, ops.ACT_NONE if last else ops.ACT_TANH, residual=before if last else None,
                                          want_f32=last, want_planes=not last, m_dev=f_dev)
        else:
            x = before
            for i, cv in enumerate(plan.postnet):
                last = i == n_post - 1
                x = ops.conv1d(x, cv.wp, cv.bias, rm.frame_lo, rm.frame_hi, ops.ACT_NONE if last else ops.ACT_TANH,
                               residual=before if last else None)
        if hp.output_activation is not None:
            x = ops.act_fwd(x, output_act_code(hp))
        utt_frames = frames_info if frames_info is not None else maps.utt_frames
        if inter is not None:
            inter.update(p_outs=p, e_outs=e, p_embs=p_emb, e_embs=e_emb, before=before, after=x, maps=maps)
            return x, utt_frames, inter
        return x, utt_frames


def synthesize(plan, xs, durs=None, f0=None, energy=None, dropout_mode=ops.DROP_RNG, prenet_keep=None, seed=0,
               bilstm_algo=0, return_intermediates=False, caps=None, spembs=None, prosody=None):
    prep = prepare(plan, xs, durs, f0, energy, device_maps=caps is not None, spembs=spembs, prosody=prosody)
    out = run(plan, prep, dropout_mode, prenet_keep, seed, bilstm_algo, return_intermediates, caps=caps)
    import os

    if bilstm_algo == 3 or os.environ.get("FCL_BILSTM_GROUP_INFER", "0") not in ("", "0"):
        ops.check_status(plan.device)
    after, utt_frames = out[0], out[1]
    if isinstance(utt_frames, DeviceFrames):
        utt_frames = utt_frames.resolve()
    mels, s = [], 0
    for n in utt_frames:
        mels.append(after[s : s + n])
        s += n
    return (mels, out[2]) if return_intermediates else mels


def predict(plan, xs, prosody=None, spembs=None, bilstm_algo=0):
    prep = prepare(plan, xs, spembs=spembs, prosody=prosody)
    with torch.cuda.device(plan.device):
        planes = use_planes(plan)
        if planes:
            hs, hs_p = encode(plan, prep, bilstm_algo, planes=True)
            predictor = lambda pp, pad: _predictor_scalar_planes(pp, hs_p, prep.seg_lo, prep.seg_hi, pad)
        else:
            hs = encode(plan, prep, bilstm_algo)
            predictor = lambda pp, pad: _predictor_scalar(pp, hs, prep.seg_lo, prep.seg_hi, pad)
        if plan.hp.spk_embed_dim is not None:
            hs, hs_p = ops.concat_spk(hs, prep.spk, prep.T, want_f32=True, want_planes=planes)
        grouped = planes and _GROUP_PREDICTORS
        m_rows = prep.B * prep.T
        p = e = None
        if grouped and plan.group_dpe is not None:
            d_log, p, e = _predictors_grouped(plan.group_dpe, hs_p, prep.seg_lo, prep.seg_hi, prep.pad, m_rows, [True, True, True])
        else:
            d_log = predictor(plan.duration, None)
        if p is None and grouped and plan.group_pe is not None:
            p, e = _predictors_grouped(plan.group_pe, hs_p, prep.seg_lo, prep.seg_hi, prep.pad, m_rows, [True, True])
        elif p is None:
            p = predictor(plan.pitch, prep.pad)
            e = predictor(plan.energy, prep.pad)
        d_int = ops.duration_round_ctl(d_log, prep.ctl, 1, False, 1.0, prep.pad)
        _, _, _, p, e = ops.variance_embed_add_ctl(None, p, e, None, None, None, None, None, None, prep.ctl, 1, want_out=False)
        d_h = d_int.view(prep.B, prep.T).cpu().numpy()
        p_h, e_h = p.view(prep.B, prep.T).cpu().numpy(), e.view(prep.B, prep.T).cpu().numpy()
    return {"duration": [d_h[b, :L].copy() for b, L in enumerate(prep.lens)], "pitch": [p_h[b, :L].copy() for b, L in enumerate(prep.lens)],
            "energy": [e_h[b, :L].copy() for b, L in enumerate(prep.lens)]}


_SHARED_STREAMS = {}


import contextlib as _contextlib


@_contextlib.contextmanager
def capture(graph, stream, pool=None):
    with torch.cuda.stream(stream):
        if pool is not None:
            graph.capture_begin(pool, capture_error_mode="global")
        else:
            graph.capture_begin(capture_error_mode="global")
        try:
            yield
        finally:
            graph.capture_end()


_PLACE_STREAMS = int(os.environ.get("FCL_PLACE_STREAMS", "1")) != 0


def shared_streams(device, n):
    dev = torch.device(device)
    key = (dev.type, dev.index if dev.index is not None else torch.cuda.current_device())
    pool = _SHARED_STREAMS.setdefault(key, [])
    if not pool:
        _SHARED_STREAMS[key + ("skipped",)] = [torch.cuda.Stream(device=dev) for _ in range(int(os.environ.get("FCL_STREAM_SKIP", "0")))]
    while len(pool) < n:
        if len(pool) < 4 and _PLACE_STREAMS:
            pool.append(ops.stream_apart(pool, device=dev))
        else:
            pool.append(torch.cuda.Stream(device=dev))
    return pool[:n]


def packed_words(frames_cap, odim, batch):
    return (int(frames_cap) * int(odim) + int(batch) + 2 + 63) // 64 * 64


class GraphRunner(object):

    def __init__(self, plan, prep, stream=None, dropout_mode=ops.DROP_RNG, seed=0, caps=None):
        self.plan, self.prep = plan, prep
        self.stream = stream if stream is not None else torch.cuda.Stream(device=plan.device)
        with torch.cuda.device(plan.device):
            self.seed_word = torch.zeros(1, dtype=torch.int32, device=plan.device)
            self.caps = caps
            with torch.cuda.stream(self.stream):
                if prep.maps is None and caps is None:
                    _, _, inter = run(plan, prep, dropout_mode, seed=seed, seed_dev=self.seed_word, return_intermediates=True)
                    self.caps = Caps.from_maps(inter["maps"])
                    self.utt_frames = list(inter["maps"].utt_frames)
                out = run(plan, prep, dropout_mode, seed=seed, seed_dev=self.seed_word, caps=self.caps)
                if isinstance(out[1], DeviceFrames):
                    self.utt_frames = out[1].resolve()
            self.stream.synchronize()
            self.graph = torch.cuda.CUDAGraph()
            with torch.cuda.graph(self.graph, stream=self.stream):
                ops.u32_add(self.seed_word, 1)
                self.mel, frames = run(plan, prep, dropout_mode, seed=seed, seed_dev=self.seed_word, caps=self.caps)
            if isinstance(frames, DeviceFrames):
                self.frames = frames
            else:
                self.frames, self.utt_frames = None, frames

    def replay(self):
        with torch.cuda.stream(self.stream):
            self.graph.replay()
        return self.mel

    def check(self):
        ops.check_status(self.plan.device)


class BatchRunner(object):

    def __init__(self, plan, batch, t_cap, caps, forced=True, stream=None, dropout_mode=ops.DROP_RNG, seed=0, depth=3, pack_outputs=False, mempool=None,
                 controls=False, tail=None):
        dev = plan.device
        self.controls = bool(controls)
        self.plan, self.B, self.T, self.caps, self.forced = plan, int(batch), int(t_cap), caps, bool(forced)
        self.S = int(plan.hp.spk_embed_dim or 0)
        self.stream = stream if stream is not None else torch.cuda.Stream(device=dev)
        n = self.B * self.T
        self._off = {}
        off = 0
        for name, nbytes in (("ids", 8 * n), ("seg_lo", 4 * n), ("seg_hi", 4 * n), ("dur", 4 * n), ("lens", 4 * ((self.B + 3) // 4 * 4)), ("pad", n),
                             ("spk", 4 * self.B * self.S), ("ctl", 4 * n * _prosody.NCTL if self.controls else 0)):
            self._off[name] = (off, nbytes)
            off += (nbytes + 15) // 16 * 16
        self._nbytes = off
        self._ingraph = os.environ.get("FCL_FEED_INGRAPH", "1") not in ("", "0")
        self._host = [torch.zeros(off, dtype=torch.uint8).pin_memory() for _ in range(1 if self._ingraph else depth)]
        self._host_ev = [None] * len(self._host)
        self._slot = 0
        self._launched = 0
        self._seq_host = torch.zeros(4, dtype=torch.int32).pin_memory()
        self._seq_np = self._seq_host.numpy()
        rows = np.arange(n, dtype=np.int32)
        self._rows = (rows // self.T, rows - (rows // self.T) * self.T, ((rows // self.T) * self.T).astype(np.int32))
        with torch.cuda.device(dev):
            self._dev = torch.zeros(off, dtype=torch.uint8, device=dev)
            view = lambda name, dt: self._dev[self._off[name][0] : self._off[name][0] + self._off[name][1]].view(dt)
            p = PreparedBatch()
            p.B, p.T, p.lens = self.B, self.T, None
            p.ids, p.seg_lo, p.seg_hi = view("ids", torch.int64), view("seg_lo", torch.int32), view("seg_hi", torch.int32)
            p.lens_dev, p.pad = view("lens", torch.int32)[: self.B], view("pad", torch.uint8)
            p.dur_pad = view("dur", torch.int32) if self.forced else None
            p.f0e, p.maps = None, None
            p.spk = view("spk", torch.float32).view(self.B, self.S) if self.S else None
            p.ctl = view("ctl", torch.float32).view(n, _prosody.NCTL) if self.controls else None
            self.prep = p
            self.seed_word = torch.zeros(1, dtype=torch.int32, device=dev)
            self.status = torch.zeros(1, dtype=torch.int32, device=dev)
            self._seq_dev = torch.zeros(1, dtype=torch.int32, device=dev)
            if self._ingraph:
                self._src_dev, self._seq_host_dev = ops.host_device_ptr(self._host[0]), ops.host_device_ptr(self._seq_host)
            self.stream.wait_stream(torch.cuda.current_stream(dev))
            self.load([np.ones(1, dtype=np.int64)] * self.B, [np.ones(1, dtype=np.int64)] * self.B if self.forced else None,
                      [np.ones(self.S, dtype=np.float32)] * self.B if self.S else None)
            warm_key = (self.B, self.T, caps.lmax, caps.frames, caps.bounds.tobytes(), caps.tail_from, self.forced, int(dropout_mode), self.S,
                        self.controls)
            warmed = plan.__dict__.setdefault("_runner_warm", set())
            if warm_key not in warmed:
                with torch.cuda.stream(self.stream):
                    if self._ingraph:
                        self._feed(False)
                    run(plan, p, dropout_mode, seed=seed, seed_dev=self.seed_word, caps=caps, status=self.status)
                self.stream.synchronize()
                if self.forced and int(self.status.item()):
                    raise ops._lib.FclError("fcl-taco2_amd: BatchRunner warm-up failed: %s" % ops.status_message(int(self.status.item()) & 0xFFFFFFFF))
                warmed.add(warm_key)
            else:
                self.stream.synchronize()
            self.status.zero_()
            self.graph = torch.cuda.CUDAGraph()
            with capture(self.graph, self.stream, mempool):
                if self._ingraph:
                    ops.feed_copy(self._dev, self._src_dev, self._nbytes, self._seq_dev, self._seq_host_dev, self.seed_word)
                else:
                    ops.u32_add(self.seed_word, 1)
                self.mel, self._frames = run(plan, p, dropout_mode, seed=seed, seed_dev=self.seed_word, caps=caps, status=self.status)
                if tail is not None:
                    tail(self)
                self.out = None
                if pack_outputs:
                    n, b1 = self.mel.numel(), self.B + 1
                    self.out = torch.empty(packed_words(self.mel.shape[0], self.mel.shape[1], self.B), dtype=torch.float32, device=dev)
                    self.out[:n].view_as(self.mel).copy_(self.mel)
                    self.out[n : n + b1].view(torch.int32).copy_(self._frames.utt_frame0[:b1])
                    self.out[n + b1 : n + b1 + 1].view(torch.int32).copy_(self.status)
        self.n_loaded = 0

    def _feed(self, bump):
        ops.feed_copy(self._dev, self._src_dev, self._nbytes, self._seq_dev, self._seq_host_dev, self.seed_word if bump else None)
        self._launched += 1

    def _wait_consumed(self):
        if int(self._seq_np[0]) == self._launched:
            return
        t0 = time.perf_counter()
        while int(self._seq_np[0]) != self._launched:
            time.sleep(0)
            if time.perf_counter() - t0 > 60.0:
                raise ops._lib.FclError("fcl-taco2_amd: BatchRunner: the feed node of launch %d never ran (sequence word %d; device hung?)"
                                        % (self._launched, int(self._seq_np[0])))

    def load(self, xs, durs=None, spembs=None, prosody=None):
        nb = len(xs)
        if prosody is not None and not self.controls:
            raise ValueError("BatchRunner: prosody controls need a runner built with controls=True")
        controls = _prosody.per_utterance(prosody, nb)
        _prosody.check_overrides(controls, forced_dur=self.forced)
        if (spembs is not None) != bool(self.S):
            raise ValueError("BatchRunner: speaker embeddings %s" % ("missing (the model has spk_embed_dim=%d)" % self.S if self.S else "given to a model without spk_embed_dim"))
        if nb > self.B or nb == 0:
            raise ValueError("BatchRunner: %d utterances, capacity %d" % (nb, self.B))
        if (durs is not None) != self.forced:
            raise ValueError("BatchRunner(forced=%s): durations %s" % (self.forced, "missing" if self.forced else "not taken (the graph predicts them)"))
        B, T, n = self.B, self.T, self.B * self.T
        as_np = lambda v: v.cpu().numpy() if torch.is_tensor(v) else np.asarray(v)
        xs = [as_np(x).reshape(-1) for x in xs]
        ln = np.fromiter((x.shape[0] for x in xs), np.int32, nb)
        if int(ln.max()) > T or int(ln.min()) < 1:
            raise ValueError("BatchRunner: utterances of %d..%d phonemes, capacity %d" % (int(ln.min()), int(ln.max()), T))
        dcat = None
        if durs is not None:
            if len(durs) != nb or any(np.asarray(d).size != k for d, k in zip(durs, ln)):
                raise ValueError("duration count != phoneme count")
            dcat = np.concatenate([np.asarray(d).reshape(-1) for d in durs])
        spk_rows = None
        if self.S:
            spk_rows = [as_np(v).reshape(-1) for v in spembs]
            if len(spk_rows) != nb or any(v.shape[0] != self.S for v in spk_rows):
                raise ValueError("BatchRunner: speaker embeddings must be %d vectors of %d values" % (nb, self.S))
        ctl_rows = _prosody.pack(controls, ln, T) if controls is not None else None
        j = self._slot % len(self._host)
        self._slot += 1
        if self._ingraph:
            self._wait_consumed()
        elif self._host_ev[j] is not None:
            self._host_ev[j].synchronize()
        hb = self._host[j].numpy()
        seg = lambda name, dt: hb[self._off[name][0] : self._off[name][0] + self._off[name][1]].view(dt)
        ids, dur, lens = seg("ids", np.int64), seg("dur", np.int32), seg("lens", np.int32)
        lens[:nb] = ln
        lens[nb:] = 0
        b_of, t_of, base = self._rows
        lfull = lens[:B][b_of]
        valid = t_of < lfull
        ids[:] = 0
        ids[valid] = np.concatenate(xs)
        if dcat is not None:
            dur[:] = 0
            dur[valid] = dcat
        if self.S:
            sp = seg("spk", np.float32).reshape(B, self.S)
            sp[nb:] = 0.0
            for i_, v in enumerate(spk_rows):
                sp[i_] = v
        if self.controls:
            ctl = seg("ctl", np.float32).reshape(n, _prosody.NCTL)
            ctl[:] = _prosody.IDENTITY
            if ctl_rows is not None:
                ctl[: nb * T] = ctl_rows
        seg("seg_lo", np.int32)[:] = base
        np.add(base, lfull, out=seg("seg_hi", np.int32))
        np.logical_not(valid, out=seg("pad", np.uint8).view(np.bool_))
        if not self._ingraph:
            with torch.cuda.stream(self.stream):
                self._dev.copy_(self._host[j], non_blocking=True)
                ev = torch.cuda.Event()
                ev.record(self.stream)
            self._host_ev[j] = ev
        self.n_loaded = nb

    def replay(self):
        with torch.cuda.stream(self.stream):
            self.graph.replay()
        self._launched += 1
        return self.mel

    def frames(self):
        self.stream.synchronize()
        self._frames._host = None
        return self._frames.resolve()[: self.n_loaded]


class SpeechRunner(BatchRunner):

    def __init__(self, plan, gen, batch, t_cap, caps, voc_frames_cap=None, forced=False, stream=None, dropout_mode=ops.DROP_RNG, seed=0, depth=3,
                 pack_outputs=False, mempool=None, controls=False):
        if int(plan.hp.odim) != int(gen.plan.A):
            raise ops._lib.FclError("fcl-taco2_amd: SpeechRunner: the model writes %d mel channels, the vocoder takes %d" % (plan.hp.odim, gen.plan.A))
        if torch.device(gen.plan.device) != torch.device(plan.device):
            raise ops._lib.FclError("fcl-taco2_amd: SpeechRunner: model and vocoder must live on one device")
        if not hasattr(gen, "capacity_synth"):
            raise ops._lib.FclError("fcl-taco2_amd: SpeechRunner: %s has no capacity form (only the Parallel WaveGAN generator can follow the synthesis pass "
                                    "inside one graph); use the two-step route (engine.run, then gen.synthesize_packed), as tts.synthesize does"
                                    % type(gen).__name__)
        self.gen, self.hop, self.seed = gen, int(gen.plan.hop), int(seed)
        with torch.cuda.device(plan.device):
            frames_cap = int(voc_frames_cap) if voc_frames_cap else caps.frames
            self.synth = gen.capacity_synth(batch, frames_cap, seed=seed)
        BatchRunner.__init__(self, plan, batch, t_cap, caps, forced=forced, stream=stream, dropout_mode=dropout_mode, seed=seed, depth=depth,
                             pack_outputs=pack_outputs, mempool=mempool, controls=controls, tail=SpeechRunner._vocoder_tail)
        self.pcm, self.live = self.synth.pcm, self.synth.live

    def _vocoder_tail(self):
        self.synth.run(self.mel, self._frames.utt_frame0, self.status, seed_dev=self.seed_word)

    def noise_seed(self):
        self.stream.synchronize()
        return (self.seed + int(self.seed_word.item())) & 0xFFFFFFFF

    def waveforms(self):
        self.stream.synchronize()
        bits = int(self.status.item()) & 0xFFFFFFFF
        if bits:
            self.status.zero_()
            raise ops._lib.FclError("fcl-taco2_amd: device status 0x%x: %s" % (bits, ops.status_message(bits)))
        f0 = self._frames.utt_frame0.cpu().numpy().astype(np.int64) * self.hop
        pcm = self.pcm[: int(f0[self.B])].cpu().numpy()
        return [pcm[int(f0[i]) : int(f0[i + 1])] for i in range(self.n_loaded)]
```

fcl-taco2_amd/ops.py:

```python
import ctypes as C

import torch

from . import _lib
from ._lib import ACT_NONE, ACT_RELU, ACT_SIGMOID, ACT_TANH, DROP_MASK, DROP_NONE, DROP_RNG, check


try:
    _raw_stream, _cur_device = torch._C._cuda_getCurrentRawStream, torch._C._cuda_getDevice
except AttributeError:
    _raw_stream = _cur_device = None


def _stream():
    if _raw_stream is not None:
        return _raw_stream(_cur_device())
    return torch.cuda.current_stream().cuda_stream


def _p(t, dtype=torch.float32):
    if t is None:
        return None
    if not t.is_cuda:
        raise _lib.FclError("fcl-taco2_amd: expected a device tensor (the HIP path has no CPU fallback)")
# ... 168 lines not shown
def conv1d_planes_group(xp, x_group_stride, wpp, bias, seg_lo, seg_hi, m, cin, cout, k, groups, act=ACT_NONE, want_f32=True, want_planes=False):
    ldxp = xp.shape[1] // 64
    y = torch.empty(groups * m, cout, device=xp.device, dtype=torch.float32) if want_f32 else None
    yp = planes_empty(groups * m, cout, xp.device) if want_planes else None
    check(_lib.load().fcl_conv1d_planes_group_fwd(_p(xp, torch.int16), ldxp, int(x_group_stride), _p(wpp, torch.int16), _p(bias), _p(seg_lo, torch.int32),
                                                  _p(seg_hi, torch.int32), _p(y), _p(yp, torch.int16), m, cin, cout, k, act, groups, _stream()))
    return y, yp


def layernorm_group(x, ldx, x_group_stride, gamma, beta, eps, m, c, groups, want_y=False, want_planes=False, lin_w=None, lin_b=None, pad_mask=None):
    y = torch.empty(groups * m, c, device=x.device, dtype=torch.float32) if want_y else None
    yp = planes_empty(groups * m, c, x.device) if want_planes else None
    scalar = torch.empty(groups * m, device=x.device, dtype=torch.float32) if lin_w is not None else None
    check(_lib.load().fcl_layernorm_group_fwd(_p(x), ldx, int(x_group_stride), _p(gamma), _p(beta), eps, _p(y), _p(yp, torch.int16), _p(lin_w), _p(lin_b),
                                              _p(pad_mask, torch.uint8), _p(scalar), m, c, groups, _stream()))
    return y, scalar, yp


def duration_round(x, linear_domain=False, offset=1.0, pad_mask=None):
    out = torch.empty(x.numel(), device=x.device, dtype=torch.int64)
    check(_lib.load().fcl_duration_round_fwd(_p(x), _p(out, torch.int64), x.numel(), int(linear_domain), offset, _p(pad_mask, torch.uint8), _stream()))
    return out


def variance_embed_add(hs, p, e, wp, bp, we, be, seg_lo, seg_hi, want_embs=False):
    m, c = hs.shape
    k = wp.shape[-1]
    out = torch.empty_like(hs)
    pe = torch.empty_like(hs) if want_embs else None
    ee = torch.empty_like(hs) if want_embs else None
    check(_lib.load().fcl_variance_embed_add_fwd(_p(hs), _p(p), _p(e), _p(wp), _p(bp), _p(we), _p(be), _p(seg_lo, torch.int32),
                                                 _p(seg_hi, torch.int32), _p(out), _p(pe), _p(ee), m, c, k, _stream()))
    return out, pe, ee


def _ctl_args(ctl, row_div):
    if ctl is None:
        return None, 0, 1
    return _p(ctl), int(ctl.shape[-1]), int(row_div)


def duration_round_ctl(x, ctl=None, ctl_row_div=1, linear_domain=False, offset=1.0, pad_mask=None):
    out = torch.empty(x.numel(), device=x.device, dtype=torch.int64)
    cp, ld, div = _ctl_args(ctl, ctl_row_div)
    check(_lib.load().fcl_duration_round_ctl_fwd(_p(x), _p(out, torch.int64), x.numel(), int(linear_domain), offset, _p(pad_mask, torch.uint8),
                                                 cp, ld, div, _stream()))
    return out


def variance_embed_add_ctl(hs, p, e, wp, bp, we, be, seg_lo, seg_hi, ctl=None, ctl_row_div=1, want_out=True, want_embs=False):
    m = p.numel()
    emb = want_out or want_embs
    c = hs.shape[1] if emb else 0
    k = wp.shape[-1] if emb else 1
    out = torch.empty_like(hs) if want_out else None
    pe = torch.empty_like(hs) if want_embs else None
    ee = torch.empty_like(hs) if want_embs else None
    p_out, e_out = torch.empty_like(p), torch.empty_like(e)
    cp, ld, div = _ctl_args(ctl, ctl_row_div)
    check(_lib.load().fcl_variance_embed_add_ctl_fwd(_p(hs) if want_out else None, _p(p), _p(e), _p(wp) if emb else None, _p(bp) if emb else None,
                                                     _p(we) if emb else None, _p(be) if emb else None, _p(seg_lo, torch.int32) if emb else None,
                                                     _p(seg_hi, torch.int32) if emb else None, cp, ld, div, _p(out), _p(pe), _p(ee), _p(p_out),
                                                     _p(e_out), m, c, k, _stream()))
    return out, pe, ee, p_out, e_out


def variance_embed_rows(hs, p, e, wp_t, bp, we_t, be, seg_lo, seg_hi, src_rows, ctl=None, ctl_row_div=1, want_scalars=False):
    m, c = hs.shape
    k, n = wp_t.shape[0], src_rows.numel()
    out_p = planes_empty(n, c, hs.device)
    p_out = torch.empty_like(p) if want_scalars else None
    e_out = torch.empty_like(e) if want_scalars else None
    cp, ld, div = _ctl_args(ctl, ctl_row_div)
    check(_lib.load().fcl_variance_embed_rows_fwd(_p(hs), _p(p), _p(e), _p(wp_t), _p(bp), _p(we_t), _p(be), _p(seg_lo, torch.int32), _p(seg_hi, torch.int32),
                                                  _p(src_rows, torch.int32), cp, ld, div, _p(out_p, torch.int16), _p(p_out), _p(e_out), m, n, c, k, _stream()))
    return out_p, p_out, e_out


def position_table(dur_i32, lmax):
    n = dur_i32.numel()
    pos = torch.empty(n, lmax, device=dur_i32.device, dtype=torch.float32)
    check(_lib.load().fcl_position_table_fwd(_p(dur_i32, torch.int32), _p(pos), n, lmax, _stream()))
    return pos


def gather_rows(src, idx_i32, want_f32=True, want_planes=False):
    n, c = idx_i32.numel(), src.shape[1]
    dst = torch.empty(n, c, device=src.device, dtype=torch.float32) if want_f32 else None
    dstp = planes_empty(n, c, src.device) if want_planes else None
    check(_lib.load().fcl_gather_rows_fwd(_p(src), _p(idx_i32, torch.int32), _p(dst), _p(dstp, torch.int16), n, c, _stream()))
    return (dst, dstp) if want_planes else dst


_STATUS = {}


def status_word(device):
    key = str(torch.device(device))
    w = _STATUS.get(key)
    if w is None:
        w = _STATUS[key] = torch.zeros(1, dtype=torch.int32, device=device)
    return w


def status_message(bits):
    msgs = []
    if bits & _lib.STATUS_GROUP_TIMEOUT:
        msgs.append("a cooperating-workgroup BiLSTM kernel timed out waiting for a group member (its outputs are partial); "
                    "it is single-stream only — run one at a time or set FCL_BILSTM_GROUP=0")
    if bits & _lib.STATUS_ZERO_DURATION:
        msgs.append("zero duration: ds_nonzeros.shape[0] != hs.shape[0] (the reference asserts on a non-padded phoneme of duration 0, "
                    "decoder_sa_kd.py:739); nothing was decoded")
    if bits & _lib.STATUS_LMAX_CAP:
        msgs.append("a duration exceeds the number of decoder steps that were launched (lmax_cap); nothing was decoded -- rerun with a larger cap")
    if bits & _lib.STATUS_FRAMES_CAP:
        msgs.append("the batch has more frames than the frame buffers hold (frames_cap); nothing was decoded -- rerun with a larger cap")
    if bits & _lib.STATUS_ROWS_CAP:
        msgs.append("a decoder step had more live rows than the host's bound for it (rows beyond the bound were not computed)")
    if bits & _lib.STATUS_VOCODER_CAP:
        msgs.append("vocoder capacity: the batch has more frames than the capacity vocoder holds (its frames_cap), or the synthesis pass in front of it "
                    "failed; no waveform was generated -- rerun with a larger vocoder frames_cap")
    if bits & _lib.STATUS_PCM_NONFINITE:
        msgs.append("the waveform holds a non-finite sample (written as 0 in the 16-bit PCM)")
    known = (_lib.STATUS_GROUP_TIMEOUT | _lib.STATUS_ZERO_DURATION | _lib.STATUS_LMAX_CAP | _lib.STATUS_FRAMES_CAP | _lib.STATUS_ROWS_CAP
             | _lib.STATUS_VOCODER_CAP | _lib.STATUS_PCM_NONFINITE)
    if bits & ~known:
        msgs.append("unknown status bits 0x%x" % (bits & ~known))
    return "; ".join(msgs)


def check_status(device, reset=True):
    w = status_word(device)
    bits = int(w.item()) & 0xFFFFFFFF
    if bits:
        if reset:
            w.zero_()
        raise _lib.FclError("fcl-taco2_amd: device status 0x%x: %s" % (bits, status_message(bits)))


def bilstm(x, lens_i32, w_ih_f, w_hh_f, b_f, w_ih_r, w_hh_r, b_r, b, t, algo=0, status=None, x_p=None, w_ih_p=None, want_planes=False, row_maps=None):
    c, dev = w_ih_f.shape[1], w_ih_f.device
    h = w_hh_f.shape[1]
    lib = _lib.load()
    nbytes = lib.fcl_bilstm_workspace_bytes(b, t, h)
    ws = torch.empty(nbytes, device=dev, dtype=torch.uint8)
    out = torch.empty(b * t, 2 * h, device=dev, dtype=torch.float32)
    outp = planes_empty(b * t, 2 * h, dev) if want_planes else None
    wf_p, wr_p = w_ih_p if (x_p is not None and w_ih_p is not None) else (None, None)
    check(lib.fcl_bilstm_fwd(_p(x), _p(lens_i32, torch.int32), _p(w_ih_f), _p(w_hh_f), _p(b_f), _p(w_ih_r), _p(w_hh_r), _p(b_r), _p(out),
                             _p(outp, torch.int16), _p(x_p if wf_p is not None else None, torch.int16), _p(wf_p, torch.int16), _p(wr_p, torch.int16),
                             b, t, c, h, algo, ws.data_ptr(), nbytes, _p(status if status is not None else status_word(dev), torch.int32),
                             C.byref(row_maps.struct) if row_maps is not None else None, _stream()))
    return (out, outp) if want_planes else out


def masked_l1_mse(a, b, row_valid, out_f64, b_log_offset=None):
    m, c = a.shape
    assert b.shape == a.shape and out_f64.dtype == torch.float64 and out_f64.numel() >= 3
    check(_lib.load().fcl_masked_l1_mse_fwd(_p(a), c, _p(b), c, _p(row_valid, torch.uint8), m, c, int(b_log_offset is not None),
                                            float(b_log_offset or 0.0), out_f64.data_ptr(), _stream()))


def u32_add(word_i32, v=1):
    check(_lib.load().fcl_u32_add(_p(word_i32, torch.int32), v, _stream()))


def host_device_ptr(pinned):
    p = _lib.load().fcl_host_device_ptr(pinned.data_ptr())
    if not p:
        msg = _lib.load().fcl_last_error()
        raise _lib.FclError("fcl-taco2_amd: %s" % (msg.decode("utf-8", "replace") if msg else "host_device_ptr failed"))
    return p


def feed_copy(dst_u8, src_devptr, nbytes, seq_dev_i32, seq_host_devptr, bump_i32=None):
    check(_lib.load().fcl_feed_copy(_p(dst_u8, torch.uint8), src_devptr, nbytes, _p(seq_dev_i32, torch.int32), seq_host_devptr, _p(bump_i32, torch.int32),
                                    _stream()))


class RowMapsRequest(object):
    __slots__ = ("maps", "struct", "_keep")


def row_maps_build(n, b, lmax_cap, frames_cap, dur_i64=None, dur_i32=None, row_src=None, utt_row0=None, t_max=0, pad=None, want_order=False,
                   status=None):
    req = row_maps_request(n, b, lmax_cap, frames_cap, dur_i64, dur_i32, row_src, utt_row0, t_max, pad, want_order, status)
    check(_lib.load().fcl_row_maps_build(C.byref(req.struct), _stream()))
    return req.maps


def row_maps_request(n, b, lmax_cap, frames_cap, dur_i64=None, dur_i32=None, row_src=None, utt_row0=None, t_max=0, pad=None, want_order=False,
                     status=None):
    ref = dur_i64 if dur_i64 is not None else dur_i32
    dev = ref.device
    sizes = dict(src_rows=n, dur=n, frame_off=n, live_rows=lmax_cap + 1, utt_frame0=b + 1, frame_lo=frames_cap, frame_hi=frames_cap, totals=4,
                 scratch=2 * n)
    if want_order:
        sizes["order"] = n
    offs, tot = {}, 0
    for k, v in sizes.items():
        offs[k] = tot
        tot += (v + 3) // 4 * 4
    blk = torch.empty(tot, dtype=torch.int32, device=dev)
    out = {k: blk[offs[k] : offs[k] + v] for k, v in sizes.items()}
    st = status if status is not None else status_word(dev)
    a = _lib.RowMaps(b=b, n=n, lmax_cap=lmax_cap, frames_cap=frames_cap, t_max=t_max, row_src=_p(row_src, torch.int32), utt_row0=_p(utt_row0, torch.int32),
                     pad=_p(pad, torch.uint8), dur_i64=_p(dur_i64, torch.int64), dur_i32=_p(dur_i32, torch.int32), src_rows=_p(out["src_rows"], torch.int32),
                     dur_sorted=_p(out["dur"], torch.int32), frame_off=_p(out["frame_off"], torch.int32),
                     order=_p(out.get("order"), torch.int32), live_rows=_p(out["live_rows"], torch.int32), utt_frame0=_p(out["utt_frame0"], torch.int32),
                     frame_lo=_p(out["frame_lo"], torch.int32), frame_hi=_p(out["frame_hi"], torch.int32), totals=_p(out["totals"], torch.int32),
                     status=st.data_ptr(), scratch=_p(out["scratch"], torch.int32))
    req = RowMapsRequest()
    req.maps, req.struct, req._keep = out, a, (blk, st, row_src, utt_row0, pad, dur_i64, dur_i32)
    return req


def decoder_loop(dw, att_c, dur_i32, live_rows, frame_off_i32, n_frames, teacher_ys=None, dropout_mode=DROP_NONE,
                 prenet_keep=None, seed=0, want_taps=False, seed_dev=None, att_c_p=None, want_before_p=False, live_rows_dev=None,
                 status=None, tail_from=0):
    lib = _lib.load()
    dev = att_c.device if att_c is not None else att_c_p.device
    n = att_c.shape[0] if att_c is not None else att_c_p.shape[0]
    lmax = int(live_rows.shape[0])
    nbytes = lib.fcl_decoder_loop_workspace_bytes(C.byref(dw.struct), n)
    ws = torch.empty(nbytes, device=dev, dtype=torch.uint8)
    before = torch.empty(n_frames, dw.struct.odim, device=dev, dtype=torch.float32)
    before_p = planes_empty(n_frames, dw.struct.odim, dev) if want_before_p else None
    if live_rows_dev is not None and status is None:
        status = status_word(dev)
    taps = None
    if want_taps:
        taps = (torch.empty(n_frames, dw.struct.p, device=dev, dtype=torch.float32),
                torch.empty(n_frames, dw.struct.u, device=dev, dtype=torch.float32),
                torch.empty(n_frames, dw.struct.u, device=dev, dtype=torch.float32))
    io = _lib.DecoderIO(
        n=n, lmax=lmax, att_c=_p(att_c), dur=_p(dur_i32, torch.int32), live_rows_host=live_rows.ctypes.data,
        frame_off=_p(frame_off_i32, torch.int32), teacher_ys=_p(teacher_ys), dropout_mode=dropout_mode,
        prenet_keep=_p(prenet_keep, torch.uint8), seed=seed & 0xFFFFFFFF, seed_dev=_p(seed_dev, torch.int32), before=_p(before),
        tap_prenet=_p(taps[0]) if taps else None, tap_lstm0=_p(taps[1]) if taps else None, tap_lstm1=_p(taps[2]) if taps else None,
        workspace=ws.data_ptr(), workspace_bytes=nbytes, att_c_p=_p(att_c_p, torch.int16), before_p=_p(before_p, torch.int16),
        live_rows=_p(live_rows_dev, torch.int32), status=None if live_rows_dev is None else status.data_ptr(), tail_from=int(tail_from))
    check(lib.fcl_decoder_loop_fwd(C.byref(dw.struct), C.byref(io), _stream()))
    res = (before, taps) if want_taps else before
    if want_before_p:
        return (res + (before_p,)) if want_taps else (res, before_p)
    return res


def gemm_tn(a, b, out, shift=0, seg_lo=None, seg_hi=None):
    m, n = a.shape
    k = b.shape[1]
    assert b.shape[0] == m and out.shape == (n, k) and out.stride(1) == 1 and out.dtype == torch.float32 and out.is_cuda
    check(_lib.load().fcl_gemm_tn_fwd(_p(a), n, _p(b), k, out.data_ptr(), out.stride(0), m, n, k, shift, _p(seg_lo, torch.int32), _p(seg_hi, torch.int32), _stream()))
    return out


def pack_planes_t(x, ntaps=1, shift0=0, seg_lo=None, seg_hi=None):
    rows, cols = x.shape
    assert x.stride(1) == 1 and rows > 0
    out = torch.empty(ntaps * cols, (rows + 31) // 32 * 64, device=x.device, dtype=torch.int16)
    assert out.data_ptr() % 128 == 0
    check(_lib.load().fcl_pack_planes_t(x.data_ptr(), x.stride(0), rows, cols, ntaps, shift0, _p(seg_lo, torch.int32), _p(seg_hi, torch.int32),
                                        _p(out, torch.int16), _stream()))
    return out


def gemm_tn_planes(ap_t, bp_t, out, m):
    n = ap_t.shape[0]
    k = bp_t.shape[0]
    if out.dim() == 3:
        ntaps, n2, kk = out.shape
        assert n2 == n and ntaps * kk == k and out.is_contiguous()
        check(_lib.load().fcl_gemm_tn_planes(_p(ap_t, torch.int16), _p(bp_t, torch.int16), out.data_ptr(), kk, m, n, k, kk, n * kk, _stream()))
    else:
        assert out.shape == (n, k) and out.stride(1) == 1
        check(_lib.load().fcl_gemm_tn_planes(_p(ap_t, torch.int16), _p(bp_t, torch.int16), out.data_ptr(), out.stride(0), m, n, k, 0, 0, _stream()))
    return out


def gemm_tn_taps(a, b, out, shift0, seg_lo=None, seg_hi=None):
    m, n = a.shape
    ntaps, n2, k = out.shape
    assert b.shape == (m, k) and n2 == n and out.is_contiguous()
    check(_lib.load().fcl_gemm_tn_taps_fwd(_p(a), n, _p(b), k, _p(out), k, m, n, k, shift0, ntaps, n * k, _p(seg_lo, torch.int32), _p(seg_hi, torch.int32),
                                           _stream()))
    return out


def l1_mse_loss_grad(a, b, row_valid, count, w_l1, w_mse, sums_f64, da=None, b_log_offset=None, want_planes=False):
    if a.dim() == 1:
        a, b = a.reshape(-1, 1), b.reshape(-1, 1)
    m, c = a.shape
    if c % 4:
        assert not want_planes
        masked_l1_mse(a, b, row_valid, sums_f64, b_log_offset)
        return l1_mse_grad(a, b, row_valid, count, w_l1, w_mse, da=da, b_log_offset=b_log_offset)
    acc = da is not None
    if da is None:
        da = torch.empty_like(a)
    dap = planes_empty(m, c, a.device) if want_planes else None
    check(_lib.load().fcl_l1_mse_loss_grad(_p(a), _p(b), _p(row_valid, torch.uint8), m, c, int(b_log_offset is not None), float(b_log_offset or 0.0),
                                           w_l1, w_mse, float(count), _p(da), int(acc), sums_f64.data_ptr(), _p(dap, torch.int16), _stream()))
    return (da, dap) if want_planes else da


def colsum(x, out, y=None, gamma=None, beta=None, mode=0, out_x=None):
# ... 460 lines not shown
```

fcl-taco2_amd/tts.py:

```python
import argparse
import logging
import os
import threading
import time
import wave

import numpy as np
import torch

from .batching import BucketStore, NullArk, Writer, chunk_selectors, take
from .decode import add_prosody_arguments, build_model, prosody_from_args, read_manifest
from .kaldi_io import ArkScpWriter
from .sharding import shard_utterances

MAX_BUCKETS = 2


def bucket_of(n_phonemes):
    return (int(n_phonemes) + 15) // 16 * 16


def plan_batches(lengths, batch_size):
    if batch_size < 1:
        raise ValueError("--batch-size must be at least 1 (got %d)" % batch_size)
    order = sorted(range(len(lengths)), key=lambda i: -int(lengths[i]))
    return [(bucket_of(max(int(lengths[i]) for i in order[s : s + batch_size])), order[s : s + batch_size]) for s in range(0, len(order), batch_size)]


def vocoder_frames_cap(caps_frames, hop):
    if int(caps_frames) * int(hop) >= 2 ** 31 - 1:
        raise ValueError("fcl-taco2_amd: a batch capacity of %d frames x hop %d exceeds 2^31 samples: use a smaller --batch-size" % (caps_frames, hop))
    return int(caps_frames)


def write_pcm_wav(path, pcm, rate):
    with wave.open(path, "wb") as w:
        w.setnchannels(1)
        w.setsampwidth(2)
        w.setframerate(int(rate))
        w.writeframes(np.ascontiguousarray(pcm, dtype="<i2").tobytes())


class _Bucket(object):

    def __init__(self, t_cap, caps):
        self.t_cap, self.caps, self.runner, self.slots, self.next, self.grow, self.copied, self.replays = t_cap, caps, None, None, 0, None, None, 0


@torch.no_grad()
def synthesize(model, gen, utts, outdir, rate, batch_size=32, seed=137, prosody=None, feats_out=None, max_buckets=None, vocoder_graph=False):
    from . import engine, ops, vocoder

    os.makedirs(outdir, exist_ok=True)
    torch.manual_seed(seed)
    dev = next(model.parameters()).device
    plan = model.plan(dev)
    hop, odim = gen.plan.hop, int(plan.hp.odim)
    if odim != gen.plan.A:
        raise ValueError("fcl-taco2_amd: the model writes %d mel channels, the vocoder takes %d" % (odim, gen.plan.A))
    spk_of, ctl_of, controlled = chunk_selectors(plan, utts, prosody)
    gen_eager = bool(getattr(gen.plan, "eager_only", False)) and not (vocoder_graph and hasattr(gen, "capacity_synth"))
    eager_only = bool(getattr(plan, "generic_decoder", False)) or plan.hp.elayers != 1 or gen_eager
    counts = dict(graph_batches=0, eager_batches=0, redone_batches=0)
    routes = {}

    def write(item):
        chunk, pcm, offs, mel, frames = item
        for i, u in enumerate(chunk):
            write_pcm_wav(os.path.join(outdir, u[0] + "_gen.wav"), pcm[offs[i] : offs[i + 1]], rate)
        if mel is not None:
            ark.write_batch([u[0] for u in chunk], mel[: int(sum(frames))], frames)

    def two_step(chunk, k):
        prep = engine.prepare(plan, [u[1] for u in chunk], spembs=spk_of(chunk), prosody=ctl_of(chunk))
        mel, frames, inter = engine.run(plan, prep, ops.DROP_RNG, seed=int(torch.randint(0, 2 ** 31 - 1, (1,)).item()), return_intermediates=True)
        frames = [int(f) for f in frames]
        nseed = (seed + 104729 * k) & 0xFFFFFFFF
        routes[k] = ("two-step", [u[0] for u in chunk], nseed)
        if hasattr(gen, "check_lens"):
            gen.check_lens(frames, [u[0] for u in chunk])
        _, flat = gen.synthesize_packed(mel, frames, seed=nseed, return_flat=True)
        offs = np.concatenate([[0], np.cumsum([gen.samples_of(f) for f in frames])])
        n = int(offs[-1])
        host = vocoder.pcm16(flat)
        wr.put((chunk, host, offs, mel.cpu().numpy() if feats_out else None, frames))
        return n, inter["maps"]

    def harvest(item):
        b, chunk, slot, ev, k = item
        ev.synchronize()
        bits = int(slot["st"][0]) & 0xFFFFFFFF
        if bits:
            slot["free"].set()
            counts["redone_batches"] += 1
            counts["graph_batches"] -= 1
            logging.info("batch %d: %s -- redone through the two-step route", k, ops.status_message(bits))
            got, b.grow = two_step(chunk, k)
            return got
        f0 = slot["f0"].numpy().astype(np.int64)
        frames = [int(v) for v in np.diff(f0[: len(chunk) + 1])]
        wr.put((chunk, slot["pcm"].numpy(), f0 * hop, slot["mel"].numpy() if feats_out else None, frames), slot["free"])
        return int(f0[len(chunk)]) * hop

    def make(t_cap, caps):
        vocoder_frames_cap(caps.frames, hop)
        return _Bucket(t_cap, caps)

    pending, samples = [], 0

    def drain(b):
        nonlocal samples
        for it in take(pending, lambda p: p[0] is b):
            samples += harvest(it)
        for sl in (b.slots or []):
            sl["free"].wait()

    store = BucketStore(engine, batch_size, make, drain, MAX_BUCKETS if max_buckets is None else max_buckets)
    with (ArkScpWriter(feats_out) if feats_out else NullArk()) as ark, torch.cuda.device(dev):
        main_stream = engine.shared_streams(dev, 1)[0]
        copy_stream = ops.stream_apart([main_stream], device=dev) if os.environ.get("FCL_PLACE_STREAMS", "1") != "0" else torch.cuda.Stream(device=dev)
        wr = Writer(write, 8)
        torch.cuda.synchronize()
        t0 = time.perf_counter()
        try:
            for k, (t_cap, idx) in enumerate(plan_batches([len(u[1]) for u in utts], batch_size)):
                chunk = [utts[i] for i in idx]
                if eager_only:
                    samples += two_step(chunk, k)[0]
                    counts["eager_batches"] += 1
                    continue
                n_ph = sum(len(u[1]) for u in chunk)
                b = store.get(t_cap, n_ph)
                if b is None:
                    got, maps = two_step(chunk, k)
                    samples += got
                    counts["eager_batches"] += 1
                    store.calibrated(t_cap, maps, n_ph)
                    continue
                if b.runner is None:
                    b.runner = engine.SpeechRunner(plan, gen, batch_size, t_cap, b.caps, forced=False, stream=main_stream, seed=seed + 31 * k,
                                                   controls=controlled)
                    r = b.runner
                    mk = lambda: dict(pcm=torch.empty(r.synth.M, dtype=torch.int16, pin_memory=True), f0=torch.empty(batch_size + 1, dtype=torch.int32, pin_memory=True),
                                      st=torch.empty(1, dtype=torch.int32, pin_memory=True), free=threading.Event(),
                                      mel=torch.empty(tuple(r.mel.shape), dtype=torch.float32, pin_memory=True) if feats_out else None)
                    b.slots = [mk(), mk()]
                    for sl in b.slots:
                        sl["free"].set()
                r = b.runner
                slot = b.slots[b.next % 2]
                b.next += 1
                for it in take(pending, lambda p: p[2] is slot):
                    samples += harvest(it)
                slot["free"].wait()
                slot["free"].clear()
                try:
                    r.load([u[1] for u in chunk], spembs=spk_of(chunk), prosody=ctl_of(chunk))
                except Exception:
                    slot["free"].set()
                    raise
                if b.copied is not None:
                    r.stream.wait_event(b.copied)
                with torch.cuda.stream(r.stream):
                    r.status.zero_()
                r.replay()
                b.replays += 1
                routes[k] = ("graph", [u[0] for u in chunk], (r.seed + b.replays) & 0xFFFFFFFF)
                done = torch.cuda.Event()
                done.record(r.stream)
                with torch.cuda.stream(copy_stream):
                    copy_stream.wait_event(done)
                    slot["pcm"].copy_(r.pcm, non_blocking=True)
                    slot["f0"].copy_(r._frames.utt_frame0[: batch_size + 1], non_blocking=True)
                    slot["st"].copy_(r.status, non_blocking=True)
                    if feats_out:
                        slot["mel"].copy_(r.mel, non_blocking=True)
                    ev = torch.cuda.Event()
                    ev.record(copy_stream)
                b.copied = ev
                pending.append((b, chunk, slot, ev, k))
                counts["graph_batches"] += 1
            while pending:
                samples += harvest(pending.pop(0))
            torch.cuda.synchronize()
        except BaseException:
            torch.cuda.synchronize()
            for it in take(pending):
                it[2]["free"].set()
            raise
        finally:
            wr.join()
        secs = time.perf_counter() - t0
        wr.close()
    audio = samples / float(rate)
    return dict(samples=int(samples), seconds=secs, rtf=secs / max(audio, 1e-9), utterances=len(utts), batches=[routes[k] for k in sorted(routes)], **counts)


def build_parser():
    from . import griffinlim

    ap = argparse.ArgumentParser(prog="fcl_taco2_amd.tts", description="FCL-taco2 text -> waveform on MI355X in one process (synthesis + Parallel WaveGAN)")
    ap.add_argument("--model", required=True)
    ap.add_argument("--model-conf", required=True)
    ap.add_argument("--teacher-config", default=None, help="model.json of the teacher (student checkpoints trained with KD projections)")
    ap.add_argument("--json", required=True, help="data.json manifest (phoneme ids per utterance)")
    ap.add_argument("--vocoder-checkpoint", default=None, help="generator checkpoint ({'model': {'generator': state_dict}} or a bare state_dict); this or "
                    "--griffin-lim")
    ap.add_argument("--griffin-lim", action="store_true", help="no vocoder checkpoint: pseudo-inverse mel filterbank + Griffin-Lim (exclusive with "
                    "--vocoder-checkpoint; every batch takes the two-step route)")
    ap.add_argument("--vocoder-config", default=None, help="parallel_wavegan config.yml (default: next to the checkpoint; v1 geometry without one)")
    ap.add_argument("--outdir", required=True)
    ap.add_argument("--feats-out", default=None, metavar="PREFIX", help="also write the mels as PREFIX.ark / PREFIX.scp")
    ap.add_argument("--batch-size", type=int, default=32)
    ap.add_argument("--max-buckets", type=int, default=MAX_BUCKETS, help="captured text->waveform graphs kept (each holds ~1.07 KB per capacity sample with "
                    "Parallel WaveGAN, ~0.94 KB with HiFi-GAN v1)")
    ap.add_argument("--vocoder-graph", action="store_true", help="HiFi-GAN: run the generator inside the captured text->waveform graph (its capacity form) "
                    "instead of the two-step route; no effect for Parallel WaveGAN, which always does")
    ap.add_argument("--nj", type=int, default=1, help="number of utterance shards (one process per GPU)")
    ap.add_argument("--job", type=int, default=0, help="this process's shard (0-based)")
    ap.add_argument("--seed", type=int, default=137)
    ap.add_argument("--verbose", type=int, default=1)
    ap.add_argument("--unsafe-pickle", action="store_true", help="allow the full unpickler for vocoder checkpoints that weights_only=True rejects (runs code "
                    "embedded in the file: trusted checkpoints only)")
    add_prosody_arguments(ap)
    griffinlim.add_arguments(ap)
    return ap


def parse_args(argv=None):
    from . import griffinlim

    ap = build_parser()
    args = ap.parse_args(argv)
    griffinlim.check_arguments(ap, args, args.vocoder_checkpoint)
    if args.batch_size < 1:
        ap.error("--batch-size must be at least 1")
    if args.nj < 1 or not 0 <= args.job < args.nj:
        ap.error("--job must lie in [0, --nj) (got --job %d --nj %d)" % (args.job, args.nj))
    if args.max_buckets < 1:
        ap.error("--max-buckets must be at least 1")
    try:
        prosody_from_args(args)
    except ValueError as e:
        ap.error(str(e))
    return args


def shard_of(utts, nj, job):
    return [utts[i] for i in shard_utterances([len(u[1]) for u in utts], nj)[job]]


def main(argv=None):
    args = parse_args(argv)
    from .vocoder_decode import build_generator

    torch.set_num_threads(4)
    logging.basicConfig(level=logging.INFO if args.verbose else logging.WARN, format="%(asctime)s %(levelname)s: %(message)s")
    dev = "cuda:%d" % (args.job % max(torch.cuda.device_count(), 1))
    model = build_model(args.model, args.model_conf, args.teacher_config, dev)
    if args.griffin_lim:
        from . import griffinlim

        gen, rate = griffinlim.from_args(args, dev, n_mels=int(model.plan(dev).hp.odim))
    else:
        gen, rate = build_generator(args.vocoder_checkpoint, dev, args.vocoder_config, args.unsafe_pickle)
    mine = shard_of(read_manifest(args.json), args.nj, args.job)
    feats = args.feats_out if args.feats_out is None or args.nj == 1 else "%s.%d" % (args.feats_out, args.job + 1)
    res = synthesize(model, gen, mine, args.outdir, rate, args.batch_size, args.seed, prosody_from_args(args, [u[0] for u in mine]), feats, args.max_buckets,
                     vocoder_graph=args.vocoder_graph)
    logging.info("generated %d utterances, %.1f s of audio in %.2f s (RTF = %.5f); batches: %d graph, %d eager, %d redone", res["utterances"],
                 res["samples"] / float(rate), res["seconds"], res["rtf"], res["graph_batches"], res["eager_batches"], res["redone_batches"])
    return res


if __name__ == "__main__":
    main()
```

include/fcl_hip.h:

```cpp
#ifndef FCL_HIP_H_
#define FCL_HIP_H_

#include <stddef.h>
#include <stdint.h>

#ifdef __cplusplus
extern "C" {
#endif

typedef void* fcl_stream_t;

enum { FCL_OK = 0, FCL_ERR_INVALID = -1, FCL_ERR_SHAPE = -2, FCL_ERR_ALIGN = -3, FCL_ERR_HIP = -4, FCL_ERR_WORKSPACE = -5 };
enum { FCL_ACT_NONE = 0, FCL_ACT_RELU = 1, FCL_ACT_TANH = 2, FCL_ACT_SIGMOID = 3 };
enum { FCL_DROP_NONE = 0, FCL_DROP_MASK = 1, FCL_DROP_RNG = 2 };
enum {
    FCL_STATUS_GROUP_TIMEOUT = 1,
    FCL_STATUS_ZERO_DURATION = 2,
    FCL_STATUS_LMAX_CAP = 4,
    FCL_STATUS_FRAMES_CAP = 8,
    FCL_STATUS_ROWS_CAP = 16,
    FCL_STATUS_VOCODER_CAP = 32,
    FCL_STATUS_PCM_NONFINITE = 64
};

enum { FCL_GEMM_F32 = 0, FCL_GEMM_BF16 = 1 };

const char* fcl_last_error(void);
#define FCL_ABI_VERSION 423
int fcl_version(void);
void* fcl_debug_ptr(void);
int fcl_set_gemm_mode(int mode);
int fcl_get_gemm_mode(void);


int fcl_pack_conv1d_weight(const float* w, const float* scale, float* out, int cout, int cin, int k, fcl_stream_t stream);

int fcl_fold_batchnorm(const float* gamma, const float* beta, const float* mean, const float* var, float eps,
                       float* scale, float* shift, int c, fcl_stream_t stream);

int fcl_copy2d(float* dst, int ld_dst, const float* src, int ld_src, int rows, int cols, fcl_stream_t stream);

int fcl_u32_add(uint32_t* p, uint32_t v, fcl_stream_t stream);

size_t fcl_frag_bf16_elems(int rows, int cols);
int fcl_pack_frag_bf16(const float* w, int rows, int cols, uint16_t* hi, uint16_t* lo, fcl_stream_t stream);
int fcl_pack_frag_f32(const float* w, int rows, int cols, float* out, fcl_stream_t stream);

size_t fcl_planes_elems(int rows, int cols);
int fcl_pack_planes(const float* x, int ld, int rows, int cols, uint16_t* out, fcl_stream_t stream);

int fcl_add_vec(const float* a, const float* b, float* out, int n, fcl_stream_t stream);

int fcl_embedding_fwd(const int64_t* ids, const float* table, float* out, uint16_t* out_p, int m, int v, int e, fcl_stream_t stream);

int fcl_embed_conv_table_fwd(const int64_t* ids, const float* tables, const float* bias, const int32_t* seg_lo, const int32_t* seg_hi,
                             const float* residual_table, float* y, uint16_t* y_p, int m, int v, int cout, int k, int act, const int32_t* m_dev,
                             fcl_stream_t stream);

int fcl_linear_fwd(const float* x, int lda, const float* w, int ldw, const float* bias, float* y, int ldy,
                   int m, int n, int k, int act, fcl_stream_t stream);

int fcl_conv1d_fwd(const float* x, const float* wp, const float* bias, const int32_t* seg_lo, const int32_t* seg_hi,
                   const float* residual, float* y, int m, int cin, int cout, int k, int act, fcl_stream_t stream);

int fcl_linear_planes_fwd(const uint16_t* xp, int ldxp, const uint16_t* wpp, const float* bias, float* y, int ldy, uint16_t* yp,
                          int m, int n, int k, int act, fcl_stream_t stream);
int fcl_linear_planes_mse_fwd(const uint16_t* xp, int ldxp, const uint16_t* wpp, const float* target, int ld_t, const uint8_t* row_valid, double count,
                              float* grad, int ldg, uint16_t* grad_p, double* sums, int m, int n, int k, fcl_stream_t stream);
int fcl_conv1d_planes_fwd(const uint16_t* xp, int ldxp, const uint16_t* wpp, const float* bias, const int32_t* seg_lo, const int32_t* seg_hi,
                          const float* residual, float* y, uint16_t* yp, int m, int cin, int cout, int k, int act, fcl_stream_t stream);
int fcl_conv1d_planes_rows_fwd(const uint16_t* xp, int ldxp, const uint16_t* wpp, const float* bias, const int32_t* seg_lo, const int32_t* seg_hi,
                               const float* residual, float* y, uint16_t* yp, int m, int cin, int cout, int k, int act, const int32_t* m_dev,
                               fcl_stream_t stream);

int fcl_conv1d_planes_bn_fwd(const uint16_t* xp, int ldxp, const uint16_t* wpp, const int32_t* seg_lo, const int32_t* seg_hi, float* z, int m, int cin, int cout, int k,
                             float eps, float momentum, float* mean, float* invstd, float* running_mean, float* running_var, double* zero_workspace,
                             fcl_stream_t stream);
int fcl_conv1d_planes_group_fwd(const uint16_t* xp, int ldxp, int64_t x_group_stride, const uint16_t* wpp, const float* bias, const int32_t* seg_lo,
                                const int32_t* seg_hi, float* y, uint16_t* yp, int m, int cin, int cout, int k, int act, int groups,
                                fcl_stream_t stream);

int fcl_layernorm_fwd(const float* x, const float* gamma, const float* beta, float eps, float* y, uint16_t* yp ,
                      const float* lin_w, const float* lin_b, const uint8_t* pad_mask, const uint8_t* keep, float keep_scale,
                      float* scalar, int m, int c, fcl_stream_t stream);
int fcl_layernorm_group_fwd(const float* x, int ldx, int64_t x_group_stride, const float* gamma, const float* beta, float eps, float* y, uint16_t* yp,
                            const float* lin_w, const float* lin_b, const uint8_t* pad_mask, float* scalar, int m, int c, int groups,
                            fcl_stream_t stream);

int fcl_duration_round_fwd(const float* x, int64_t* out, int n, int linear_domain, float offset,
                           const uint8_t* pad_mask, fcl_stream_t stream);

int fcl_variance_embed_add_fwd(const float* hs, const float* p, const float* e, const float* wp, const float* bp,
                               const float* we, const float* be, const int32_t* seg_lo, const int32_t* seg_hi,
                               float* out, float* p_emb, float* e_emb, int m, int c, int k, fcl_stream_t stream);

int fcl_duration_round_ctl_fwd(const float* x, int64_t* out, int n, int linear_domain, float offset, const uint8_t* pad_mask, const float* ctl,
                               int ctl_ld, int ctl_row_div, fcl_stream_t stream);
int fcl_variance_embed_add_ctl_fwd(const float* hs, const float* p, const float* e, const float* wp, const float* bp, const float* we,
                                   const float* be, const int32_t* seg_lo, const int32_t* seg_hi, const float* ctl, int ctl_ld, int ctl_row_div,
                                   float* out, float* p_emb, float* e_emb, float* p_out, float* e_out, int m, int c, int k, fcl_stream_t stream);
int fcl_variance_embed_rows_fwd(const float* hs, const float* p, const float* e, const float* wp_t, const float* bp, const float* we_t, const float* be,
                                const int32_t* seg_lo, const int32_t* seg_hi, const int32_t* src_rows, const float* ctl, int ctl_ld, int ctl_row_div,
                                uint16_t* out_p, float* p_out, float* e_out, int m, int n, int c, int k, fcl_stream_t stream);

int fcl_concat_spk_fwd(const float* hs, int ldh, const float* spk, float* out, uint16_t* out_p, int m, int c, int s, int t, fcl_stream_t stream);

int fcl_position_table_fwd(const int32_t* dur, float* pos, int n, int lmax, fcl_stream_t stream);

int fcl_gather_rows_fwd(const float* src, const int32_t* idx, float* dst, uint16_t* dst_p, int n, int c, fcl_stream_t stream);

struct fcl_row_maps;
size_t fcl_bilstm_workspace_bytes(int b, int t, int h);
int fcl_bilstm_fwd(const float* x, const int32_t* lens, const float* w_ih_f, const float* w_hh_f, const float* b_f,
                   const float* w_ih_r, const float* w_hh_r, const float* b_r, float* out, uint16_t* out_p, const uint16_t* x_p,
                   const uint16_t* w_ih_f_p, const uint16_t* w_ih_r_p, int b, int t, int c, int h,
                   int algo, void* workspace, size_t workspace_bytes, uint32_t* status, const struct fcl_row_maps* row_maps, fcl_stream_t stream);

typedef struct {
    const float* A;
    const float* W;
    int lda, ldw, K;
    int shift;
    const uint16_t* Whi;
    const uint16_t* Wlo;
    const uint16_t* Ap;
    const uint16_t* Wp;
    int lda_p, ldw_p;
    int64_t a_chunk_stride;
    const float* Wff;
} fcl_gemm_term_t;

typedef struct {
    fcl_gemm_term_t term[3];
    int nterms;
    int M, U;
    const float* G;
    long long g_row_mul, g_row_add;
    const float* bias;
    const float* rank1_w;
    const int32_t* dur;
    int step;
    const float* h_in;
    float* h_out;
    float* c;
    float zoneout;
    const uint8_t* zone_keep_h;
    const uint8_t* zone_keep_c;
    const int32_t* row_len;
    float* out2;
    const int32_t* out2_row_base;
    long long out2_row_mul, out2_row_add;
    int ld2, out2_col_off;
    uint16_t* h_out_p;
    int ld_hp;
    float* save_gates;
    float* save_c_new;
    float* save_c_old;
    float* save_h_old;
    const int32_t* m_dev;
} fcl_lstm_step_t;

int fcl_lstm_step_fwd(const fcl_lstm_step_t* args, fcl_stream_t stream);

typedef struct {
    int c;
    int p;
    int u;
    int odim;
    const float* prenet_w0;
    const float* prenet_b0;
    const float* prenet_w1;
    const float* prenet_b1;
    const float* w0_att;
    const float* w0_pre;
    const float* w0_pos;
    const float* w0_hh;
    const float* b0;
    const float* w1_ih;
    const float* w1_hh;
    const float* b1;
    const float* wf_h;
    const float* wf_att;
    float zoneout_rate;
    float prenet_dropout;
    const uint16_t *prenet_w0_hi, *prenet_w0_lo, *prenet_w1_hi, *prenet_w1_lo;
    const uint16_t *w0_pre_hi, *w0_pre_lo, *w0_hh_hi, *w0_hh_lo, *w1_ih_hi, *w1_ih_lo, *w1_hh_hi, *w1_hh_lo;
    const uint16_t *wf_h_hi, *wf_h_lo;
    const uint16_t *w0_att_p, *wf_att_p, *w0_pre_p, *w0_hh_p, *w1_ih_p, *w1_hh_p;
    int out_act;
    const float *wf_h_ff, *prenet_w0_ff, *prenet_w1_ff;
    const float *w0_pre_ff, *w0_hh_ff, *w1_ih_ff, *w1_hh_ff;
    const uint16_t* stream;
    int prenet_layers;
    int dlayers;
    const float *prenet_w2, *prenet_b2, *w2_ih, *w2_hh, *b2;
    int reduction_factor;
} fcl_decoder_weights_t;

typedef struct {
    int n;
    int lmax;
    const float* att_c;
    const int32_t* dur;
    const int32_t* live_rows_host;
    const int32_t* frame_off;
    const float* teacher_ys;
    int dropout_mode;
    const uint8_t* prenet_keep;
    uint32_t seed;
    const uint32_t* seed_dev;
    float* before;
    float* tap_prenet;
    float* tap_lstm0;
    float* tap_lstm1;
    void* workspace;
    size_t workspace_bytes;
    const uint16_t* att_c_p;
    uint16_t* before_p;
    const int32_t* live_rows;
    uint32_t* status;
    int tail_from;
} fcl_decoder_io_t;

size_t fcl_decoder_loop_workspace_bytes(const fcl_decoder_weights_t* w, int n);
size_t fcl_decoder_stream_bytes(const fcl_decoder_weights_t* w);
int fcl_decoder_stream_pack(const fcl_decoder_weights_t* w, void* out, size_t out_bytes, fcl_stream_t stream);
int fcl_decoder_loop_fwd(const fcl_decoder_weights_t* w, const fcl_decoder_io_t* io, fcl_stream_t stream);

typedef struct fcl_row_maps {
    int b, n;
    int lmax_cap, frames_cap;
    int t_max;
    const int32_t* row_src;
    const int32_t* utt_row0;
    const uint8_t* pad;
    const int64_t* dur_i64;
    const int32_t* dur_i32;
    int32_t* src_rows;
    int32_t* dur_sorted;
    int32_t* frame_off;
    int32_t* order;
    int32_t* live_rows;
    int32_t* utt_frame0;
    int32_t* frame_lo;
    int32_t* frame_hi;
    int32_t* totals;
    uint32_t* status;
    int32_t* scratch;
} fcl_row_maps_t;
int fcl_row_maps_build(const fcl_row_maps_t* maps, fcl_stream_t stream);

int fcl_masked_l1_mse_fwd(const float* a, int lda, const float* b, int ldb, const uint8_t* row_valid, int m, int c,
                          int b_log, float b_log_offset, double* out, fcl_stream_t stream);

int fcl_gemm_tn_fwd(const float* a, int lda, const float* b, int ldb, float* c, int ldc, int m, int n, int k, int shift,
                    const int32_t* seg_lo, const int32_t* seg_hi, fcl_stream_t stream);
int fcl_gemm_tn_taps_fwd(const float* a, int lda, const float* b, int ldb, float* c, int ldc, int m, int n, int k, int shift0, int ntaps,
                         size_t c_tap_stride, const int32_t* seg_lo, const int32_t* seg_hi, fcl_stream_t stream);
int fcl_pack_planes_t(const float* x, int ld, int rows, int cols, int ntaps, int shift0, const int32_t* seg_lo, const int32_t* seg_hi, uint16_t* out,
                      fcl_stream_t stream);
int fcl_gemm_tn_planes(const uint16_t* ap_t, const uint16_t* bp_t, float* c, int ldc, int m, int n, int k, int nblk, size_t blk_stride,
                       fcl_stream_t stream);
int fcl_colsum_fwd(const float* x, const float* y, const float* g, const float* b, float* out, int m, int c, int mode, fcl_stream_t stream);
int fcl_colsum2_fwd(const float* x, const float* y, const float* g, const float* b, float* out, float* out_x, int m, int c, int mode, fcl_stream_t stream);
int fcl_conv1d_in1_dw(const float* dy, int ldy, const float* x, const int32_t* seg_lo, const int32_t* seg_hi, float* dw, float* db, int m, int c, int k,
                      fcl_stream_t stream);
int fcl_add2d(float* dst, int ld_dst, const float* src, int ld_src, int rows, int cols, float alpha, const uint8_t* row_valid, fcl_stream_t stream);
int fcl_act_fwd(const float* x, const uint8_t* keep, float keep_scale, float* y, uint16_t* yp, int cols, size_t n, int act, fcl_stream_t stream);
int fcl_unpack_conv1d_grad(const float* dwp, const float* scale, float* dw, int cout, int cin, int k, fcl_stream_t stream);
// ... 530 lines not shown
```

Measured before the change: 52.65 million.

## Pack encoder phoneme rows compactly instead of padding every utterance to T

```diff
diff --git a/fcl-taco2_amd/_lib.py b/fcl-taco2_amd/_lib.py
--- a/fcl-taco2_amd/_lib.py
+++ b/fcl-taco2_amd/_lib.py
@@ -260,6 +260,8 @@
     "fcl_gather_rows_fwd": (_I, [_P, _P, _P, _P, _I, _I, _P]),
     "fcl_bilstm_workspace_bytes": (_Z, [_I, _I, _I]),
     "fcl_bilstm_fwd": (_I, [_P] * 13 + [_I, _I, _I, _I, _I, _P, _Z, _P, _P, _P]),
+    "fcl_bilstm_rows_workspace_bytes": (_Z, [_I, _I]),
+    "fcl_bilstm_rows_fwd": (_I, [_P] * 14 + [_I, _I, _I, _I, _P, _Z, _P, _P]),
     "fcl_decoder_loop_workspace_bytes": (_Z, [C.POINTER(DecoderWeights), _I]),
     "fcl_decoder_stream_bytes": (_Z, [C.POINTER(DecoderWeights)]),
     "fcl_decoder_stream_pack": (_I, [C.POINTER(DecoderWeights), _P, _Z, _P]),
diff --git a/fcl-taco2_amd/batching.py b/fcl-taco2_amd/batching.py
--- a/fcl-taco2_amd/batching.py
+++ b/fcl-taco2_amd/batching.py
@@ -15,7 +15,9 @@
     bounds[: maps.lmax] = live
     bounds[maps.lmax :] = live[-1]
     bounds = np.maximum.accumulate(bounds[::-1])[::-1].astype(np.int32)
-    return engine.Caps(lmax, (int(maps.n_frames * scale) + 255) // 256 * 256, bounds, tail_from=maps.lmax + 2)
+    caps = engine.Caps(lmax, (int(maps.n_frames * scale) + 255) // 256 * 256, bounds, tail_from=maps.lmax + 2)
+    caps.rows = int(live[0])
+    return caps
 
 
 class _ScaledMaps(object):
diff --git a/fcl-taco2_amd/csrc/bilstm.hip b/fcl-taco2_amd/csrc/bilstm.hip
--- a/fcl-taco2_amd/csrc/bilstm.hip
+++ b/fcl-taco2_amd/csrc/bilstm.hip
@@ -144,12 +144,14 @@
     return o;
 }
 
-template <bool SAVE = false, bool MAPS = false>
+template <bool SAVE = false, bool MAPS = false, bool ROWS = false>
 __global__ __launch_bounds__(512) void bilstm_ksplit_kernel(const float* __restrict__ gx_f, const float* __restrict__ gx_r,
                                                             const float* __restrict__ whh_f, const float* __restrict__ whh_r,
                                                             const int* __restrict__ lens, float* __restrict__ out, int T, BilstmSave sv = BilstmSave(),
-                                                            unsigned short* __restrict__ out_p = nullptr, fcl_row_maps_t mp = fcl_row_maps_t()) {
+                                                            unsigned short* __restrict__ out_p = nullptr, fcl_row_maps_t mp = fcl_row_maps_t(),
+                                                            const int* __restrict__ utt_row0 = nullptr) {
     constexpr int H = 128;
+    static_assert(!(ROWS && SAVE), "the training forward keeps the padded layout");
     if constexpr (MAPS) {
         if (blockIdx.x == gridDim.x - 1) {
             if (blockIdx.y == 0) {
@@ -164,9 +166,11 @@
     const int b = blockIdx.x, dir = blockIdx.y, j = threadIdx.x;
     const int q = j & 7, R = j >> 3;
     const int g = q & 3, U = 2 * R + (q >> 2);
-    const float* gx = (dir ? gx_r : gx_f) + (size_t)b * T * (4 * H);
+    const int nutt = (int)gridDim.x - (MAPS ? 1 : 0);
+    const int row0 = ROWS ? min(max(utt_row0[b], 0), T) : b * T;
+    const float* gx = (dir ? gx_r : gx_f) + (size_t)row0 * (4 * H);
     const float* whh = dir ? whh_r : whh_f;
-    const int len = lens[b];
+    const int len = ROWS ? max(min(lens[b], T - row0), 0) : lens[b];
 
     f32x2 w[4][16];
 #pragma unroll
@@ -181,9 +185,10 @@
         }
     }
     if (j < 2 * H) (&h_s[0][0])[j] = 0.f;
-    for (int t = len + (j / H); t < T; t += 4) {
-        out[((size_t)b * T + t) * (2 * H) + dir * H + (j % H)] = 0.f;
-        if (out_p) store_p32(out_p, (2 * H + 31) >> 5, b * T + t, dir * H + (j % H), 0.f);
+    const int z0 = ROWS ? min(max(utt_row0[nutt], 0), T) + 4 * b : row0 + len, z1 = ROWS ? T : row0 + T, zs = ROWS ? 4 * nutt : 4;
+    for (int r = z0 + (j / H); r < z1; r += zs) {
+        out[(size_t)r * (2 * H) + dir * H + (j % H)] = 0.f;
+        if (out_p) store_p32(out_p, (2 * H + 31) >> 5, r, dir * H + (j % H), 0.f);
     }
     __syncthreads();
 
@@ -217,8 +222,8 @@
             }
             if (g == 0) {
                 h_s[(d & 1) ^ 1][U] = h;
-                out[((size_t)b * T + t) * (2 * H) + dir * H + U] = h;
-                if (out_p) store_p32(out_p, (2 * H + 31) >> 5, b * T + t, dir * H + U, h);
+                out[((size_t)row0 + t) * (2 * H) + dir * H + U] = h;
+                if (out_p) store_p32(out_p, (2 * H + 31) >> 5, row0 + t, dir * H + U, h);
             }
             c = c_new;
             h_prev = h;
@@ -968,4 +973,64 @@
     return after.finish(out_p ? fcl_pack_planes(out, 2 * h, b * t, 2 * h, out_p, stream) : 0);
 }
 
-}
+size_t fcl_bilstm_rows_workspace_bytes(int n_rows, int h) {
+    if (n_rows <= 0 || h <= 0) return 0;
+    return sizeof(float) * ((size_t)2 * n_rows * 4 * h) + 256;
+}
+
+int fcl_bilstm_rows_fwd(const float* x, const int32_t* lens, const int32_t* utt_row0, const float* w_ih_f, const float* w_hh_f, const float* b_f,
+                        const float* w_ih_r, const float* w_hh_r, const float* b_r, float* out, uint16_t* out_p, const uint16_t* x_p,
+                        const uint16_t* w_ih_f_p, const uint16_t* w_ih_r_p, int b, int n_rows, int c, int h, void* workspace, size_t workspace_bytes,
+                        const fcl_row_maps_t* row_maps, fcl_stream_t stream) {
+    FCL_REQUIRE((x || x_p) && lens && utt_row0 && w_ih_f && w_hh_f && b_f && w_ih_r && w_hh_r && b_r && out, FCL_ERR_INVALID, "bilstm_rows_fwd: null argument");
+    FCL_REQUIRE((x_p == nullptr) == (w_ih_f_p == nullptr) && (x_p == nullptr) == (w_ih_r_p == nullptr), FCL_ERR_INVALID,
+                "bilstm_rows_fwd: x_p / w_ih_f_p / w_ih_r_p come together");
+    FCL_REQUIRE(b > 0 && n_rows > 0 && c > 0 && (c & 3) == 0, FCL_ERR_SHAPE, "bilstm_rows_fwd: bad sizes B=%d rows=%d C=%d", b, n_rows, c);
+    FCL_REQUIRE(h == 128, FCL_ERR_SHAPE, "bilstm_rows_fwd: H=%d: the compact row layout covers H = 128 (fcl_bilstm_fwd takes the padded layout)", h);
+    FCL_REQUIRE(workspace && workspace_bytes >= fcl_bilstm_rows_workspace_bytes(n_rows, h), FCL_ERR_WORKSPACE, "bilstm_rows_fwd: workspace too small");
+    FCL_REQUIRE(aligned16(workspace) && aligned16(out), FCL_ERR_ALIGN, "bilstm_rows_fwd: 16-byte alignment required");
+    bool maps_fusable = false;
+    if (row_maps) {
+        const int rc = row_maps_check(row_maps, &maps_fusable);
+        if (rc) return rc;
+        FCL_REQUIRE(row_maps->n == n_rows && row_maps->b == b && row_maps->utt_row0 && !row_maps->row_src, FCL_ERR_INVALID,
+                    "bilstm_rows_fwd: the row maps take the same compact universe (n = rows, utt_row0, no row_src)");
+    }
+    const bool fuse = row_maps && maps_fusable;
+    FCL_REQUIRE(fuse ? ks_claims_simd(bilstm_ksplit_kernel<false, true, true>, "bilstm_ksplit_kernel<false, true, true>")
+                     : ks_claims_simd(bilstm_ksplit_kernel<false, false, true>, "bilstm_ksplit_kernel<false, false, true>"),
+                FCL_ERR_INVALID, "bilstm_rows_fwd: the lane-split kernel is off in this build");
+    hipStream_t s = (hipStream_t)stream;
+    float* gx_f = reinterpret_cast<float*>(workspace);
+    float* gx_r = gx_f + (size_t)n_rows * 4 * h;
+    for (int d = 0; d < 2; ++d) {
+        GemmArgs g = {};
+        g.term[0] = GemmTerm{x, d ? w_ih_r : w_ih_f, c, c, c, 0};
+        if (x_p) {
+            g.term[0].Ap = x_p;
+            g.term[0].Wp = d ? w_ih_r_p : w_ih_f_p;
+            g.term[0].lda_p = g.term[0].ldw_p = (c + 31) / 32;
+        }
+        g.nterms = 1;
+        g.M = n_rows;
+        g.N = 4 * h;
+        g.bias = d ? b_r : b_f;
+        g.Y = d ? gx_r : gx_f;
+        g.ldy = 4 * h;
+        int rc = launch_gemm(g, s);
+        if (rc) return rc;
+    }
+    {
+        ProfScope ps(fuse ? "bilstm_ksplit_kernel+maps/rows" : "bilstm_ksplit_kernel/rows", 2.0 * 2 * (double)n_rows * 4 * h * h, (double)n_rows, s);
+        if (fuse)
+            hipLaunchKernelGGL((bilstm_ksplit_kernel<false, true, true>), dim3(b + 1, 2), dim3(512), 0, s, gx_f, gx_r, w_hh_f, w_hh_r, lens, out, n_rows,
+                               BilstmSave(), out_p, *row_maps, utt_row0);
+        else
+            hipLaunchKernelGGL((bilstm_ksplit_kernel<false, false, true>), dim3(b, 2), dim3(512), 0, s, gx_f, gx_r, w_hh_f, w_hh_r, lens, out, n_rows,
+                               BilstmSave(), out_p, fcl_row_maps_t(), utt_row0);
+    }
+    const int rc = check_hip(hipGetLastError(), "bilstm k-split (rows) launch");
+    return (fuse || rc || !row_maps) ? rc : fcl_row_maps_build(row_maps, stream);
+}
+
+}
diff --git a/fcl-taco2_amd/decode.py b/fcl-taco2_amd/decode.py
--- a/fcl-taco2_amd/decode.py
+++ b/fcl-taco2_amd/decode.py
@@ -214,6 +214,11 @@
                 for it in take(pending, lambda p: p[1] == j):
                     frames += harvest(it)
                 r = pool.runner(j)
+                if r.R is not None and n_ph > r.R:
+                    n_redo += 1
+                    got, pool.grow = eager(chunk)
+                    frames += got
+                    continue
                 slot = pool.slots[j][(pool.next // len(streams)) % 2]
                 slot.free.wait()
                 slot.free.clear()
diff --git a/fcl-taco2_amd/engine.py b/fcl-taco2_amd/engine.py
--- a/fcl-taco2_amd/engine.py
+++ b/fcl-taco2_amd/engine.py
@@ -104,16 +104,18 @@
 
 class PreparedBatch(object):
     __slots__ = ("B", "T", "lens", "ids", "seg_lo", "seg_hi", "pad", "lens_dev", "f0e", "maps", "src_rows", "dur", "frame_off",
-                 "frame_lo", "frame_hi", "dur_pad", "spk", "ctl")
+                 "frame_lo", "frame_hi", "dur_pad", "spk", "ctl", "n_rows", "utt_row0", "rows_total")
 
 
 class Caps(object):
-    __slots__ = ("lmax", "frames", "bounds", "tail_from")
-
-    def __init__(self, lmax, frames, bounds, tail_from=0):
+    __slots__ = ("lmax", "frames", "bounds", "tail_from", "rows")
+
+    def __init__(self, lmax, frames, bounds, tail_from=0, rows=None):
         self.lmax, self.frames = int(lmax), int(frames)
         self.bounds = np.ascontiguousarray(np.asarray(bounds, dtype=np.int32))
         self.tail_from = int(tail_from) if 0 < int(tail_from) < self.lmax else 0
+        self.rows = int(rows) if rows is not None else None
+        assert self.rows is None or self.rows > 0
         assert self.bounds.shape == (self.lmax,) and self.lmax > 0 and self.frames > 0
 
     @staticmethod
@@ -126,7 +128,8 @@
         bounds = np.ones(lmax, dtype=np.int32)
         for m in host_maps:
             bounds[: m.lmax] = np.maximum(bounds[: m.lmax], m.live_rows)
-        return Caps(lmax, (max(m.n_frames for m in host_maps) + frame_round - 1) // frame_round * frame_round, bounds)
+        return Caps(lmax, (max(m.n_frames for m in host_maps) + frame_round - 1) // frame_round * frame_round, bounds,
+                    rows=max(int(m.src_rows.shape[0]) for m in host_maps))
 
     @staticmethod
     def generous(n_rows, lmax, frames):
@@ -159,6 +162,10 @@
 
 _GROUP_PREDICTORS = _os.environ.get("FCL_PRED_GROUP", "1") not in ("", "0")
 _VAR_EMBED_ROWS = _os.environ.get("FCL_VAR_EMBED_ROWS", "1") not in ("", "0")
+
+
+def compact_rows_enabled():
+    return _os.environ.get("FCL_COMPACT_ROWS", "1") not in ("", "0")
 
 
 def _ring():
@@ -249,21 +256,29 @@
     bl = plan.blstm
     res = plan.hp.use_residual
     convs, tabs = plan.enc_convs, getattr(plan, "embed_conv_tables", None)
+    n_rows = getattr(prep, "n_rows", None)
+    m_dev = prep.rows_total if n_rows is not None else None
     if tabs is not None:
         x, xp = ops.embed_conv_table(prep.ids, tabs, convs[0].bias, prep.seg_lo, prep.seg_hi, ops.ACT_RELU, residual_table=plan.embed if res else None,
-                                     want_f32=res or not planes, want_planes=planes)
+                                     want_f32=res or not planes, want_planes=planes, m_dev=m_dev)
         convs = convs[1:]
     if planes:
         if tabs is None:
             x, xp = ops.embedding(prep.ids, plan.embed, want_f32=res, want_planes=True)
         for cv in convs:
-            x, xp = ops.conv1d_planes(xp, cv, prep.seg_lo, prep.seg_hi, ops.ACT_RELU, residual=x if res else None, want_f32=res)
+            x, xp = ops.conv1d_planes(xp, cv, prep.seg_lo, prep.seg_hi, ops.ACT_RELU, residual=x if res else None, want_f32=res, m_dev=m_dev)
+        if n_rows is not None:
+            return ops.bilstm_rows(None, prep.lens_dev, prep.utt_row0, bl["w_ih_f"], bl["w_hh_f"], bl["b_f"], bl["w_ih_r"], bl["w_hh_r"], bl["b_r"], prep.B,
+                                   n_rows, x_p=xp, w_ih_p=(bl["w_ih_p_f"], bl["w_ih_p_r"]), want_planes=True, row_maps=row_maps)
         return ops.bilstm(None, prep.lens_dev, bl["w_ih_f"], bl["w_hh_f"], bl["b_f"], bl["w_ih_r"], bl["w_hh_r"], bl["b_r"], prep.B, prep.T, bilstm_algo,
                           x_p=xp, w_ih_p=(bl["w_ih_p_f"], bl["w_ih_p_r"]), want_planes=True, row_maps=row_maps)
     if tabs is None:
         x = ops.embedding(prep.ids, plan.embed)
     for cv in convs:
         x = ops.conv1d(x, cv.wp, cv.bias, prep.seg_lo, prep.seg_hi, ops.ACT_RELU, residual=x if res else None)
+    if n_rows is not None:
+        return ops.bilstm_rows(x, prep.lens_dev, prep.utt_row0, bl["w_ih_f"], bl["w_hh_f"], bl["b_f"], bl["w_ih_r"], bl["w_hh_r"], bl["b_r"], prep.B, n_rows,
+                               row_maps=row_maps)
     for i, bl in enumerate(plan.blstm_layers):
         x = ops.bilstm(x, prep.lens_dev, bl["w_ih_f"], bl["w_hh_f"], bl["b_f"], bl["w_ih_r"], bl["w_hh_r"], bl["b_r"], prep.B, prep.T, bilstm_algo,
                        row_maps=row_maps if i == 0 else None)
@@ -286,8 +301,12 @@
         planes = use_planes(plan)
         hs_p = None
         maps_req = None
+        n_univ = getattr(prep, "n_rows", None)
+        utt_row0 = prep.utt_row0 if n_univ is not None else None
+        if n_univ is None:
+            n_univ = prep.B * prep.T
         if prep.maps is None and prep.dur_pad is not None and caps is not None:
-            maps_req = ops.row_maps_request(prep.B * prep.T, prep.B, caps.lmax, caps.frames, dur_i32=prep.dur_pad, t_max=prep.T, pad=prep.pad,
+            maps_req = ops.row_maps_request(n_univ, prep.B, caps.lmax, caps.frames, dur_i32=prep.dur_pad, utt_row0=utt_row0, t_max=prep.T, pad=prep.pad,
                                             status=status)
         if planes:
             hs, hs_p = encode(plan, prep, bilstm_algo, planes=True, row_maps=maps_req)
@@ -299,12 +318,13 @@
         if hp.spk_embed_dim is not None:
             if getattr(prep, "spk", None) is None:
                 raise ValueError("fcl-taco2_amd: this pass needs speaker embeddings (prepare(..., spembs=...))")
+            assert utt_row0 is None, "concat_spk finds the utterance as row // T: speaker models keep the padded layout"
             hs, hs_p = ops.concat_spk(hs, prep.spk, prep.T, want_f32=True, want_planes=planes)
         rm = prep
         frames_info = None
         ctl = getattr(prep, "ctl", None)
         grouped = planes and prep.f0e is None and _GROUP_PREDICTORS
-        m_rows = prep.B * prep.T
+        m_rows = n_univ
         p = e = None
         if prep.maps is None:
             d_int = None
@@ -320,8 +340,8 @@
                 if inter is not None:
                     inter["d_log"], inter["d_int"] = d_log, d_int
             if caps is not None:
-                dm = maps_req.maps if maps_req is not None else ops.row_maps_build(prep.B * prep.T, prep.B, caps.lmax, caps.frames, dur_i64=d_int,
-                                                                                   t_max=prep.T, pad=prep.pad, status=status)
+                dm = maps_req.maps if maps_req is not None else ops.row_maps_build(n_univ, prep.B, caps.lmax, caps.frames, dur_i64=d_int,
+                                                                                   utt_row0=utt_row0, t_max=prep.T, pad=prep.pad, status=status)
                 rm = PreparedBatch()
                 rm.maps = _DevMaps(dm, caps)
                 rm.src_rows, rm.dur, rm.frame_off, rm.frame_lo, rm.frame_hi = dm["src_rows"], dm["dur"], dm["frame_off"], dm["frame_lo"], dm["frame_hi"]
@@ -329,6 +349,7 @@
             else:
                 if d_int is None:
                     raise ValueError("prepare(device_maps=True) leaves the row maps to the device: run() needs caps")
+                assert utt_row0 is None, "compact rows come with capacities (BatchRunner)"
                 d_host = d_int.cpu().numpy().reshape(prep.B, prep.T)
                 rm = PreparedBatch()
                 _upload_maps(rm, build_row_maps(prep.lens, [d_host[b, : prep.lens[b]] for b in range(prep.B)], prep.T, hp.reduction_factor), dev)
@@ -523,23 +544,14 @@
         self.plan, self.B, self.T, self.caps, self.forced = plan, int(batch), int(t_cap), caps, bool(forced)
         self.S = int(plan.hp.spk_embed_dim or 0)
         self.stream = stream if stream is not None else torch.cuda.Stream(device=dev)
-        n = self.B * self.T
-        self._off = {}
-        off = 0
-        for name, nbytes in (("ids", 8 * n), ("seg_lo", 4 * n), ("seg_hi", 4 * n), ("dur", 4 * n), ("lens", 4 * ((self.B + 3) // 4 * 4)), ("pad", n),
-                             ("spk", 4 * self.B * self.S), ("ctl", 4 * n * _prosody.NCTL if self.controls else 0)):
-            self._off[name] = (off, nbytes)
-            off += (nbytes + 15) // 16 * 16
-        self._nbytes = off
-        self._ingraph = os.environ.get("FCL_FEED_INGRAPH", "1") not in ("", "0")
-        self._host = [torch.zeros(off, dtype=torch.uint8).pin_memory() for _ in range(1 if self._ingraph else depth)]
-        self._host_ev = [None] * len(self._host)
-        self._slot = 0
-        self._launched = 0
-        self._seq_host = torch.zeros(4, dtype=torch.int32).pin_memory()
-        self._seq_np = self._seq_host.numpy()
-        rows = np.arange(n, dtype=np.int32)
-        self._rows = (rows // self.T, rows - (rows // self.T) * self.T, ((rows // self.T) * self.T).astype(np.int32))
+        rows = None
+        if (compact_rows_enabled() and caps.rows is not None and self.B <= caps.rows < self.B * self.T and not self.S and plan.hp.elayers == 1
+                and not getattr(plan, "generic_decoder", False) and int(plan.blstm["w_hh_f"].shape[1]) == 128):
+            rows = int(caps.rows)
+        self._host_init(rows, depth)
+        if self.R is not None:
+            caps = self.caps = Caps(caps.lmax, caps.frames, np.minimum(caps.bounds, self.R), caps.tail_from, self.R)
+        n, off = self.R if self.R is not None else self.B * self.T, self._nbytes
         with torch.cuda.device(dev):
             self._dev = torch.zeros(off, dtype=torch.uint8, device=dev)
             view = lambda name, dt: self._dev[self._off[name][0] : self._off[name][0] + self._off[name][1]].view(dt)
@@ -551,6 +563,9 @@
             p.f0e, p.maps = None, None
             p.spk = view("spk", torch.float32).view(self.B, self.S) if self.S else None
             p.ctl = view("ctl", torch.float32).view(n, _prosody.NCTL) if self.controls else None
+            if self.R is not None:
+                p.n_rows = self.R
+                p.utt_row0, p.rows_total = view("row0", torch.int32)[: self.B + 1], view("row0", torch.int32)[self.B + 1 : self.B + 2]
             self.prep = p
             self.seed_word = torch.zeros(1, dtype=torch.int32, device=dev)
             self.status = torch.zeros(1, dtype=torch.int32, device=dev)
@@ -561,7 +576,7 @@
             self.load([np.ones(1, dtype=np.int64)] * self.B, [np.ones(1, dtype=np.int64)] * self.B if self.forced else None,
                       [np.ones(self.S, dtype=np.float32)] * self.B if self.S else None)
             warm_key = (self.B, self.T, caps.lmax, caps.frames, caps.bounds.tobytes(), caps.tail_from, self.forced, int(dropout_mode), self.S,
-                        self.controls)
+                        self.controls, self.R)
             warmed = plan.__dict__.setdefault("_runner_warm", set())
             if warm_key not in warmed:
                 with torch.cuda.stream(self.stream):
@@ -593,6 +608,29 @@
                     self.out[n + b1 : n + b1 + 1].view(torch.int32).copy_(self.status)
         self.n_loaded = 0
 
+    def _host_init(self, rows, depth, pin=True):
+        self.R = rows
+        n = self.R if self.R is not None else self.B * self.T
+        self._off = {}
+        off = 0
+        for name, nbytes in (("ids", 8 * n), ("seg_lo", 4 * n), ("seg_hi", 4 * n), ("dur", 4 * n), ("lens", 4 * ((self.B + 3) // 4 * 4)), ("pad", n),
+                             ("spk", 4 * self.B * self.S), ("ctl", 4 * n * _prosody.NCTL if self.controls else 0),
+                             ("row0", 4 * (self.B + 2) if self.R is not None else 0)):
+            self._off[name] = (off, nbytes)
+            off += (nbytes + 15) // 16 * 16
+        self._nbytes = off
+        self._ingraph = os.environ.get("FCL_FEED_INGRAPH", "1") not in ("", "0")
+        pinned = (lambda t: t.pin_memory()) if pin else (lambda t: t)
+        self._host = [pinned(torch.zeros(off, dtype=torch.uint8)) for _ in range(1 if self._ingraph else depth)]
+        self._host_ev = [None] * len(self._host)
+        self._slot = 0
+        self._launched = 0
+        self._seq_host = pinned(torch.zeros(4, dtype=torch.int32))
+        self._seq_np = self._seq_host.numpy()
+        rows = np.arange(self.B * self.T, dtype=np.int32)
+        self._rows = (rows // self.T, rows - (rows // self.T) * self.T, ((rows // self.T) * self.T).astype(np.int32))
+        self.n_loaded = 0
+
     def _feed(self, bump):
         ops.feed_copy(self._dev, self._src_dev, self._nbytes, self._seq_dev, self._seq_host_dev, self.seed_word if bump else None)
         self._launched += 1
@@ -625,6 +663,9 @@
         ln = np.fromiter((x.shape[0] for x in xs), np.int32, nb)
         if int(ln.max()) > T or int(ln.min()) < 1:
             raise ValueError("BatchRunner: utterances of %d..%d phonemes, capacity %d" % (int(ln.min()), int(ln.max()), T))
+        total = int(ln.sum())
+        if self.R is not None and total > self.R:
+            raise ValueError("BatchRunner: %d phonemes in the batch, row capacity %d (caps.rows)" % (total, self.R))
         dcat = None
         if durs is not None:
             if len(durs) != nb or any(np.asarray(d).size != k for d, k in zip(durs, ln)):
@@ -647,6 +688,21 @@
         ids, dur, lens = seg("ids", np.int64), seg("dur", np.int32), seg("lens", np.int32)
         lens[:nb] = ln
         lens[nb:] = 0
+        if self.R is not None:
+            self._pack_compact(seg, xs, ln, total, dcat, ctl_rows)
+        else:
+            self._pack_padded(seg, xs, nb, dcat, spk_rows, ctl_rows)
+        if not self._ingraph:
+            with torch.cuda.stream(self.stream):
+                self._dev.copy_(self._host[j], non_blocking=True)
+                ev = torch.cuda.Event()
+                ev.record(self.stream)
+            self._host_ev[j] = ev
+        self.n_loaded = nb
+
+    def _pack_padded(self, seg, xs, nb, dcat, spk_rows, ctl_rows):
+        B, T, n = self.B, self.T, self.B * self.T
+        ids, dur, lens = seg("ids", np.int64), seg("dur", np.int32), seg("lens", np.int32)
         b_of, t_of, base = self._rows
         lfull = lens[:B][b_of]
         valid = t_of < lfull
@@ -668,13 +724,31 @@
         seg("seg_lo", np.int32)[:] = base
         np.add(base, lfull, out=seg("seg_hi", np.int32))
         np.logical_not(valid, out=seg("pad", np.uint8).view(np.bool_))
-        if not self._ingraph:
-            with torch.cuda.stream(self.stream):
-                self._dev.copy_(self._host[j], non_blocking=True)
-                ev = torch.cuda.Event()
-                ev.record(self.stream)
-            self._host_ev[j] = ev
-        self.n_loaded = nb
+
+    def _pack_compact(self, seg, xs, ln, total, dcat, ctl_rows):
+        B, T, R, nb = self.B, self.T, self.R, ln.shape[0]
+        row0 = seg("row0", np.int32)
+        row0[0] = 0
+        np.cumsum(ln, out=row0[1 : nb + 1])
+        row0[nb + 1 :] = total
+        ids, dur = seg("ids", np.int64), seg("dur", np.int32)
+        ids[:total] = np.concatenate(xs)
+        ids[total:] = 0
+        if dcat is not None:
+            dur[:total] = dcat
+            dur[total:] = 0
+        lo, hi, pad = seg("seg_lo", np.int32), seg("seg_hi", np.int32), seg("pad", np.uint8)
+        lo[:total] = np.repeat(row0[:nb], ln)
+        hi[:total] = np.repeat(row0[1 : nb + 1], ln)
+        lo[total:] = 0
+        hi[total:] = 0
+        pad[:total] = 0
+        pad[total:] = 1
+        if self.controls:
+            ctl = seg("ctl", np.float32).reshape(R, _prosody.NCTL)
+            ctl[:] = _prosody.IDENTITY
+            if ctl_rows is not None:
+                ctl[:total] = ctl_rows[(np.arange(T, dtype=np.int32)[None, :] < ln[:, None]).reshape(-1)]
 
     def replay(self):
         with torch.cuda.stream(self.stream):
diff --git a/fcl-taco2_amd/ops.py b/fcl-taco2_amd/ops.py
--- a/fcl-taco2_amd/ops.py
+++ b/fcl-taco2_amd/ops.py
@@ -344,6 +344,26 @@
                              b, t, c, h, algo, ws.data_ptr(), nbytes, _p(status if status is not None else status_word(dev), torch.int32),
                              C.byref(row_maps.struct) if row_maps is not None else None, _stream()))
     return (out, outp) if want_planes else out
+
+
+def bilstm_rows(x, lens_i32, utt_row0_i32, w_ih_f, w_hh_f, b_f, w_ih_r, w_hh_r, b_r, b, n_rows, x_p=None, w_ih_p=None, want_planes=False, row_maps=None,
+                out=None, out_p=None):
+    c, dev = w_ih_f.shape[1], w_ih_f.device
+    h = w_hh_f.shape[1]
+    lib = _lib.load()
+    assert utt_row0_i32.numel() >= b + 1 and lens_i32.numel() >= b
+    nbytes = lib.fcl_bilstm_rows_workspace_bytes(n_rows, h)
+    ws = torch.empty(nbytes, device=dev, dtype=torch.uint8)
+    if out is None:
+        out = torch.empty(n_rows, 2 * h, device=dev, dtype=torch.float32)
+    outp = out_p if out_p is not None else (planes_empty(n_rows, 2 * h, dev) if want_planes else None)
+    assert out.shape[0] >= n_rows and out.shape[1] == 2 * h and (outp is None or outp.shape[0] >= n_rows)
+    wf_p, wr_p = w_ih_p if (x_p is not None and w_ih_p is not None) else (None, None)
+    check(lib.fcl_bilstm_rows_fwd(_p(x), _p(lens_i32, torch.int32), _p(utt_row0_i32, torch.int32), _p(w_ih_f), _p(w_hh_f), _p(b_f), _p(w_ih_r), _p(w_hh_r),
+                                  _p(b_r), _p(out), _p(outp, torch.int16), _p(x_p if wf_p is not None else None, torch.int16), _p(wf_p, torch.int16),
+                                  _p(wr_p, torch.int16), b, n_rows, c, h, ws.data_ptr(), nbytes,
+                                  C.byref(row_maps.struct) if row_maps is not None else None, _stream()))
+    return (out, outp) if (want_planes or out_p is not None) else out
 
 
 def masked_l1_mse(a, b, row_valid, out_f64, b_log_offset=None):
diff --git a/fcl-taco2_amd/tts.py b/fcl-taco2_amd/tts.py
--- a/fcl-taco2_amd/tts.py
+++ b/fcl-taco2_amd/tts.py
@@ -148,6 +148,12 @@
                     for sl in b.slots:
                         sl["free"].set()
                 r = b.runner
+                if r.R is not None and n_ph > r.R:
+                    counts["redone_batches"] += 1
+                    logging.info("batch %d: %d phonemes, row capacity %d -- redone through the two-step route", k, n_ph, r.R)
+                    got, b.grow = two_step(chunk, k)
+                    samples += got
+                    continue
                 slot = b.slots[b.next % 2]
                 b.next += 1
                 for it in take(pending, lambda p: p[2] is slot):
diff --git a/include/fcl_hip.h b/include/fcl_hip.h
--- a/include/fcl_hip.h
+++ b/include/fcl_hip.h
@@ -115,6 +115,11 @@
                    const float* w_ih_r, const float* w_hh_r, const float* b_r, float* out, uint16_t* out_p, const uint16_t* x_p,
                    const uint16_t* w_ih_f_p, const uint16_t* w_ih_r_p, int b, int t, int c, int h,
                    int algo, void* workspace, size_t workspace_bytes, uint32_t* status, const struct fcl_row_maps* row_maps, fcl_stream_t stream);
+size_t fcl_bilstm_rows_workspace_bytes(int n_rows, int h);
+int fcl_bilstm_rows_fwd(const float* x, const int32_t* lens, const int32_t* utt_row0, const float* w_ih_f, const float* w_hh_f, const float* b_f,
+                        const float* w_ih_r, const float* w_hh_r, const float* b_r, float* out, uint16_t* out_p, const uint16_t* x_p,
+                        const uint16_t* w_ih_f_p, const uint16_t* w_ih_r_p, int b, int n_rows, int c, int h, void* workspace, size_t workspace_bytes,
+                        const struct fcl_row_maps* row_maps, fcl_stream_t stream);
 
 typedef struct {
     const float* A;
```

After: 54.03 million (median of 6 runs). +2.6%, better.
